# Sue1347/SMSUT-MedicalImgSegmentation

Measured on AMD Instinct MI355X. Metric: slices/sec uganConsisTrainer step @256x256, higher is better.
Workload: dtype f32

## Files before the change

include/smsut_hip.h:

```cpp
#ifndef SMSUT_HIP_H
#define SMSUT_HIP_H

#include <stdint.h>

#ifdef __cplusplus
extern "C" {
#endif

int smsut_conv2d_fwd_generic(const float* x, const float* w, const float* bias , float* y, int N, int H,
                             int W, int Cin, int Ho, int Wo, int Cout, int KH, int KW, int stride, int pad,
                             void* stream);
int smsut_conv2d_dgrad_generic(const float* gy, const float* w, float* gx, int N, int H, int W, int Cin, int Ho, int Wo,
                               int Cout, int KH, int KW, int stride, int pad, void* stream);
int64_t smsut_conv2d_wgrad_generic_ws(int N, int Ho, int Wo, int Cin, int Cout, int KH, int KW);
int smsut_conv2d_wgrad_generic(const float* x, const float* gy, float* gw, float* workspace, int N, int H, int W,
                               int Cin, int Ho, int Wo, int Cout, int KH, int KW, int stride, int pad, void* stream);

int smsut_conv2d_mfma_supported(int KS, int stride, int pad, int Kdim, int Ndim);
int smsut_conv2d_fwd_mfma(const float* x, const float* w, float* y, int N, int H, int W, int Kdim, int Ndim, int KS,
                          int transposed, void* stream);
int smsut_conv2d_mfma_tiles(int N, int H, int W, int Kdim, int Ndim, int KS, int f16);
int smsut_conv2d_mfma_persistent(int N, int H, int W, int Kdim, int Ndim, int KS, int f16);
int smsut_conv2d_dgrad_mfma_bwdstats(const float* gy, const float* w, float* gz, float* stats, const float* y1,
                                     const float* mean, const float* rstd, const float* gamma, const float* beta,
                                     float slope, int N, int H, int W, int Kdim, int Ndim, void* stream);
int smsut_conv2d_fwd_mfma_stats(const float* x, const float* w, float* y, float* stats, int N, int H, int W, int Kdim,
                                int Ndim, int KS, void* stream);
int smsut_conv2d_fwd_mfma_cfg(const float* x, const float* w, float* y, int N, int H, int W, int Kdim, int Ndim, int KS,
                              int transposed, int cfg, void* stream);
int64_t smsut_wino_image_floats(int Kdim, int Ndim);
int smsut_wino_prepare(const float* const* w, float* const* u, const int* Kdim, const int* Ndim, const int* transposed, int count,
                       void* stream);
int smsut_conv2d_fwd_mfma_pre(const float* x, const float* w, float* y, int N, int H, int W, int Kdim, int Ndim, int KS,
                              int transposed, const float* wu, void* stream);
int smsut_conv2d_fwd_mfma_stats_pre(const float* x, const float* w, float* y, float* stats, int N, int H, int W, int Kdim,
                                    int Ndim, int KS, const float* wu, void* stream);
int smsut_conv2d_dgrad_mfma_bwdstats_pre(const float* gy, const float* w, float* gz, float* stats, const float* y1,
                                         const float* mean, const float* rstd, const float* gamma, const float* beta,
                                         float slope, int N, int H, int W, int Kdim, int Ndim, const float* wu, void* stream);
int smsut_conv2d_fwd_mfma_stats_inaff_pre(const float* x, const float* w, float* y, float* stats, const float* mean,
                                          const float* rstd, const float* gamma, const float* beta, float slope, int N, int H,
                                          int W, int Kdim, int Ndim, const float* wu, void* stream);
int smsut_conv2d_fwd_mfma_stats_cat_pre(const float* xa, const float* xb, const float* w, float* y, float* stats, int N, int H,
                                        int W, int Kdim, int Ndim, const float* wu, void* stream);
int smsut_conv2d_fwd_mfma_split_pre(const float* x, const float* w, float* ya, float* yb, int split, int N, int H, int W,
                                    int Kdim, int Ndim, int transposed, const float* wu, void* stream);
int smsut_conv2d_fwd_mfma_stats_sc_pre(const float* x, const float* xb, const float* w, const float* wsc, float* y, float* ysc,
                                       float* stats, float* stats_sc, int N, int H, int W, int Kdim, int Ndim, const float* wu,
                                       void* stream);
int smsut_conv2d_wgrad_mfma_supported(int KS, int stride, int pad, int Cin, int Cout);
int64_t smsut_conv2d_wgrad_mfma_ws(int N, int H, int W, int Cin, int Cout, int KS);
int smsut_conv2d_wgrad_mfma(const float* x, const float* gy, float* gw, float* workspace, int N, int H, int W, int Cin,
                            int Cout, int KS, void* stream);

int smsut_conv1x1_supported(int Kdim, int Ndim);
int smsut_conv1x1_tiles(int N, int HW, int Ndim);
int smsut_conv1x1_fwd(const float* x, const float* w, float* y, float* stats , int N, int HW, int Kdim,
                      int Ndim, int transposed, void* stream);
int64_t smsut_conv1x1_wgrad_ws(int N, int HW, int Cin, int Cout);
int smsut_conv1x1_wgrad(const float* x, const float* gy, float* gw, float* workspace, int N, int HW, int Cin, int Cout,
                        void* stream);

int smsut_conv2d_fwd_mfma_stats_inaff(const float* x, const float* w, float* y, float* stats, const float* mean,
                                      const float* rstd, const float* gamma, const float* beta, float slope, int N, int H,
                                      int W, int Kdim, int Ndim, void* stream);
int smsut_conv2d_wgrad_mfma_inaff(const float* x, const float* gy, float* gw, float* workspace, const float* mean,
                                  const float* rstd, const float* gamma, const float* beta, float slope, int N, int H, int W,
                                  int Cin, int Cout, void* stream);
int smsut_conv2d_wgrad_mfma_slabs(const float* x, const float* gy, float* workspace, const float* mean, const float* rstd,
                                  const float* gamma, const float* beta, float slope, int N, int H, int W, int Cin, int Cout,
                                  void* stream);
int smsut_conv2d_mfma_form(int N, int H, int W, int Kdim, int Ndim, int sc_dgrad);

int smsut_conv2d_mfma_cat_supported(int N, int H, int W, int Kdim, int Ndim);
int smsut_conv2d_fwd_mfma_stats_cat(const float* xa, const float* xb, const float* w, float* y, float* stats, int N, int H,
                                    int W, int Kdim, int Ndim, void* stream);
int smsut_conv2d_fwd_sc_supported(int N, int H, int W, int Kdim, int Ndim, int cat);
int smsut_conv2d_fwd_mfma_stats_sc(const float* x, const float* xb , const float* w, const float* wsc, float* y,
                                   float* ysc, float* stats, float* stats_sc, int N, int H, int W, int Kdim, int Ndim,
                                   void* stream);
int smsut_conv2d_fwd_sc_f16_supported(int N, int H, int W, int Kdim, int Ndim, int cat);
int smsut_conv2d_fwd_mfma_stats_sc_f16(const float* x, const float* xb, const float* w, const float* wsc, float* y, float* ysc,
                                       float* stats, float* stats_sc, int N, int H, int W, int Kdim, int Ndim, void* stream);
int smsut_conv2d_dgrad_sc_supported(int N, int H, int W, int Cout, int Cin, int split);
int smsut_conv2d_dgrad_mfma_sc(const float* gy, const float* gs, const float* w, const float* wsc, float* gxa,
                               float* gxb , int split, int N, int H, int W, int Cout, int Cin, void* stream);
int smsut_conv2d_wgrad_sc_supported(int N, int H, int W, int Cin, int Cout);
int64_t smsut_conv2d_wgrad_sc_ws(int N, int H, int W, int Cin, int Cout);
int smsut_conv2d_wgrad_mfma_sc(const float* xa, const float* xb , int ca, const float* gy, const float* gs,
                               float* gw10, float* workspace, int N, int H, int W, int Cin, int Cout, void* stream);
int smsut_conv2d_wgrad_mfma_cat(const float* xa, const float* xb, int ca, const float* gy, float* gw, float* workspace,
                                int N, int H, int W, int Cin, int Cout, int KS, void* stream);
int smsut_conv2d_fwd_mfma_stats_sc_fin(const float* x, const float* xb , const float* w, const float* wsc, float* y,
                                       float* ysc, float* stats, float* stats_sc, int* tickets, float* mean, float* rstd,
                                       float* mean_sc, float* rstd_sc, float eps, int N, int H, int W, int Kdim, int Ndim,
                                       const float* wu , void* stream);
int smsut_conv2d_fwd_mfma_stats_inaff_fin(const float* x, const float* w, float* y, float* stats, const float* mean,
                                          const float* rstd, const float* gamma, const float* beta, float slope, int* tickets,
                                          float* mean_out, float* rstd_out, float eps, int N, int H, int W, int Kdim, int Ndim,
                                          const float* wu , void* stream);
int smsut_conv2d_dgrad_mfma_bwdstats_fin(const float* gy, const float* w, float* gz, float* stats, const float* y1,
                                         const float* mean, const float* rstd, const float* gamma, const float* beta, float slope,
                                         int* tickets, float* a_mean, float* b_mean, int N, int H, int W, int Kdim, int Ndim,
                                         const float* wu , void* stream);
int smsut_conv2d_wgrad_pair_supported(int NA, int NB, int H, int W, int Cin, int Cout, int cat, int aff, int sc);
int64_t smsut_conv2d_wgrad_pair_ws(int NA, int NB, int H, int W, int Cin, int Cout, int cat, int aff, int sc);
int smsut_conv2d_wgrad_pair(const float* xA, const float* x2A , const float* gyA, const float* gsA ,
                            const float* meanA , const float* rstdA , int NA, const float* xB,
                            const float* x2B , const float* gyB, const float* gsB ,
                            const float* meanB , const float* rstdB , int NB, int ca,
                            const float* gamma , const float* beta , float slope, float* gw, float* workspace,
                            int H, int W, int Cin, int Cout, void* stream);
int smsut_conv2d_wgrad_pair_slabs(const float* xA, const float* gyA, const float* meanA , const float* rstdA ,
                                  int NA, const float* xB, const float* gyB, const float* meanB ,
                                  const float* rstdB , int NB, const float* gamma , const float* beta ,
                                  float slope, float* workspace, int H, int W, int Cin, int Cout, void* stream);
int smsut_conv1x1_fwd_cat(const float* xa, const float* xb, int ca, const float* w, float* y, float* stats ,
                          int N, int HW, int Kdim, int Ndim, void* stream);
int smsut_conv1x1_wgrad_cat(const float* xa, const float* xb, int ca, const float* gy, float* gw, float* workspace, int N,
                            int HW, int Cin, int Cout, void* stream);

int smsut_conv2d_mfma_split_supported(int N, int H, int W, int Kdim, int Ndim, int split);
int smsut_conv2d_fwd_mfma_split(const float* x, const float* w, float* ya, float* yb, int split, int N, int H, int W,
                                int Kdim, int Ndim, int transposed, void* stream);
int smsut_conv1x1_fwd_split(const float* x, const float* w, float* ya, float* yb, int split, int N, int HW, int Kdim,
                            int Ndim, int transposed, void* stream);

int smsut_conv2d_f16_supported(int KS, int Kdim, int Ndim);
int smsut_conv2d_fwd_mfma_f16(const float* x, const float* w, float* y, const float* gsc , int N, int H, int W,
                              int Kdim, int Ndim, int KS, int transposed, void* stream);
int smsut_conv2d_fwd_mfma_stats_f16(const float* x, const float* w, float* y, float* stats, int N, int H, int W, int Kdim,
                                    int Ndim, int KS, void* stream);
int smsut_conv2d_fwd_mfma_stats_cat_f16(const float* xa, const float* xb, const float* w, float* y, float* stats, int N, int H,
                                        int W, int Kdim, int Ndim, void* stream);
int smsut_conv2d_fwd_mfma_split_f16(const float* x, const float* w, float* ya, float* yb, const float* gsc ,
                                    int split, int N, int H, int W, int Kdim, int Ndim, int transposed, void* stream);
int smsut_conv2d_f16_hs_supported(int N, int H, int W, int Kdim, int Ndim, int cat);
int smsut_conv2d_fwd_mfma_stats_f16_hs(const float* x, const float* xb , const float* w, void* y16, float* stats, int N,
                                       int H, int W, int Kdim, int Ndim, void* stream);
int smsut_conv2d_fwd_mfma_stats_f16_hsx(const void* x16, const float* w, void* y16, float* stats, int N, int H, int W, int Kdim,
                                        int Ndim, void* stream);
int smsut_conv2d_fwd_mfma_stats_inaff_f16_hsx(const void* y1_16, const float* w, void* y16, float* stats, const float* mean,
                                              const float* rstd, const float* gamma, const float* beta, float slope, int N, int H,
                                              int W, int Kdim, int Ndim, void* stream);
int smsut_conv2d_fwd_mfma_stats_sc_f16_hs(const float* x, const float* xb , const float* w, const float* wsc, void* y16,
                                          void* ysc16, float* stats, float* stats_sc, int N, int H, int W, int Kdim, int Ndim,
                                          void* stream);
int smsut_conv2d_dgrad_mfma_bwdstats_f16_hs(const float* gy, const float* w, float* gz, float* stats, const void* y1_16,
                                            const float* mean, const float* rstd, const float* gamma, const float* beta,
                                            const float* gsc , float slope, int N, int H, int W, int Kdim, int Ndim,
                                            void* stream);
int smsut_conv2d_dgrad_sc_f16_supported(int N, int H, int W, int Cout, int Cin, int split);
int smsut_conv2d_dgrad_mfma_sc_f16(const float* gy, const float* gs, const float* w, const float* wsc, float* gxa,
                                   float* gxb , const float* gsc, int split, int N, int H, int W, int Cout, int Cin,
                                   void* stream);
int smsut_conv2d_dgrad_mfma_bwdstats_f16(const float* gy, const float* w, float* gz, float* stats, const float* y1,
                                         const float* mean, const float* rstd, const float* gamma, const float* beta,
                                         const float* gsc , float slope, int N, int H, int W, int Kdim, int Ndim,
                                         void* stream);
int smsut_conv2d_wgrad_f16_supported(int N, int H, int W, int Cin, int Cout);
int64_t smsut_conv2d_wgrad_f16_ws(int N, int H, int W, int Cin, int Cout);
int smsut_conv2d_wgrad_f16(const float* x, const float* x2 , int ca, const float* gy, float* gw, float* workspace,
                           const float* gsc , int N, int H, int W, int Cin, int Cout, void* stream);
int smsut_conv2d_wgrad_f16_xh(const void* x16, const float* gy, float* gw, float* workspace, const float* gsc , int N,
                              int H, int W, int Cin, int Cout, void* stream);
int smsut_conv2d_wgrad_f16_xh_inaff(const void* y1_16, const float* gy, float* gw, float* workspace, const float* gsc ,
                                    const float* mean, const float* rstd, const float* gamma, const float* beta, float slope, int N,
                                    int H, int W, int Cin, int Cout, void* stream);
int smsut_conv2d_wgrad_sc_f16_supported(int N, int H, int W, int Cin, int Cout);
int64_t smsut_conv2d_wgrad_sc_f16_ws(int N, int H, int W, int Cin, int Cout);
int smsut_conv2d_wgrad_sc_f16(const float* x, const float* x2 , int ca, const float* gy, const float* gs, float* gw10,
                              float* workspace, const float* gsc, int N, int H, int W, int Cin, int Cout, void* stream);
int64_t smsut_absmax_scale_ws(int64_t n);
int smsut_absmax_scale(const float* x, int64_t n, float* out2, float* workspace, void* stream);
int smsut_absmax_scale2(const float* x, int64_t n, const float* x2, int64_t n2, float* out2, float* workspace, void* stream);
int smsut_absmax_finish(const float* amax, int n, float* out2, void* stream);

int smsut_conv2d_k4_supported(int Cin, int Cout);
int smsut_conv2d_k4_fwd(const float* x, const float* w, float* y, int N, int H, int W, int Cin, int Cout, int transposed,
                        void* stream);
int64_t smsut_conv2d_k4_wgrad_ws(int N, int H, int W, int Cin, int Cout);
int smsut_conv2d_k4_wgrad(const float* x, const float* gy, float* gw, float* workspace, int N, int H, int W, int Cin, int Cout,
                          void* stream);

int smsut_conv1x1_thin_supported(int Cin, int Cout);
int smsut_conv1x1_thin_dgrad(const float* gy, const float* w, float* gx, int N, int HW, int Cin, int Cout, void* stream);
int64_t smsut_conv1x1_thin_wgrad_ws(int Cin);
int smsut_conv1x1_thin_wgrad(const float* x, const float* gy, float* gw, float* workspace, int N, int HW, int Cin,
                             int Cout, void* stream);

int smsut_conv2d_small_supported(int KS, int Cin, int Cout);
int smsut_conv2d_small_fwd(const float* x, const float* w, const float* bias , float* y, int N, int H, int W,
                           int Cin, int Ho, int Wo, int Cout, int KS, int stride, int pad, void* stream);
int smsut_conv2d_small_dgrad(const float* gy, const float* w, float* gx, int N, int H, int W, int Cin, int Ho, int Wo,
                             int Cout, int KS, int stride, int pad, void* stream);
int smsut_conv2d_flat_wgrad_supported(int KS, int stride, int Cin, int Cout);
int64_t smsut_conv2d_flat_wgrad_ws(int N, int Ho, int Wo, int Cin, int Cout, int KS);
int smsut_conv2d_flat_wgrad(const float* x, const float* gy, float* gw, float* workspace, int N, int H, int W, int Cin,
                            int Ho, int Wo, int Cout, int KS, int stride, int pad, void* stream);

int smsut_convT2x2_mfma_supported(int Cin, int Cout);
int smsut_convT2x2_fwd_mfma(const float* x, const float* w, float* y, int N, int H, int W, int Cin, int Cout, void* stream);
int smsut_convT2x2_dgrad_mfma(const float* gy, const float* w, float* gx, int N, int H, int W, int Cin, int Cout,
                              void* stream);
int64_t smsut_convT2x2_wgrad_mfma_ws(int N, int H, int W, int Cin, int Cout);
int smsut_convT2x2_wgrad_mfma(const float* x, const float* gy, float* gw, float* workspace, int N, int H, int W, int Cin,
                              int Cout, void* stream);
int smsut_convT2x2_ps_supported(int Cin, int Cout);
int smsut_convT2x2_fwd_ps(const float* x, const float* w, float* y, int N, int H, int W, int Cin, int Cout, void* stream);
int64_t smsut_convT2x2_wgrad_ps_ws(int N, int H, int W, int Cin, int Cout);
int smsut_convT2x2_wgrad_ps(const float* x, const float* gy, float* gw, float* workspace, int N, int H, int W, int Cin,
                            int Cout, void* stream);

int64_t smsut_colsum_ws(int64_t rows, int C);
int smsut_colsum(const float* x, float* out, float* workspace, int64_t rows, int C, void* stream);

int smsut_in_chunks(int N, int HW, int C);
int smsut_in_slabs(int N, int HW, int C);
int smsut_instnorm_fwd(const float* x, const float* gamma, const float* beta, float* y, float* mean, float* rstd,
                       float* workspace, int N, int HW, int C, float eps, float slope, int has_act, void* stream);
int smsut_instnorm_fwd_partials(const float* x, const float* gamma, const float* beta, float* y, float* mean,
                                float* rstd, const float* partials, int chunks, int N, int HW, int C, float eps,
                                float slope, int has_act, void* stream);
int smsut_instnorm_fwd_partials_hs(const void* x16, const float* gamma, const float* beta, float* y, float* mean,
                                   float* rstd, const float* partials, int chunks, int N, int HW, int C, float eps,
                                   float slope, int has_act, void* stream);
int smsut_instnorm_fwd_partials_hs2(const void* x16, const float* gamma, const float* beta, void* y16, float* mean,
                                    float* rstd, const float* partials, int chunks, int N, int HW, int C, float eps,
                                    float slope, int has_act, void* stream);
int smsut_in_finalize_fwd(const float* partials, int chunks, float* mean, float* rstd, int N, int HW, int C, float eps,
                          void* stream);
int smsut_in_finalize_fwd2(const float* pa, int chunks_a, float* mean_a, float* rstd_a, const float* pb, int chunks_b, float* mean_b,
                           float* rstd_b, int N, int HW, int C, float eps, void* stream);
int smsut_in_finalize_bwd(const float* partials, int chunks, float* a_mean, float* b_mean, int N, int HW, int C, void* stream);
int smsut_in_apply_bwd(const float* gz, const float* x, const float* mean, const float* rstd, const float* gamma,
                       const float* a_mean, const float* b_mean, float* gx, float* ggamma ,
                       float* gbeta , int N, int HW, int C, void* stream);
int smsut_amax_blocks(int N, int HW, int C);
int smsut_in_apply_bwd_amax(const float* gz, const float* x, const float* mean, const float* rstd, const float* gamma,
                            const float* a_mean, const float* b_mean, float* gx, float* ggamma ,
                            float* gbeta , float* amax, int N, int HW, int C, void* stream);
int smsut_in_apply_bwd_hs(const float* gz, const void* x16, const float* mean, const float* rstd, const float* gamma,
                          const float* a_mean, const float* b_mean, float* gx, float* ggamma ,
                          float* gbeta , float* amax , int N, int HW, int C, void* stream);
int smsut_restail_fwd(const float* y2, const float* m2, const float* r2, const float* g2, const float* b2, const float* s,
                      const float* ms , const float* rs, const float* gs, const float* bs, float* out,
                      int N, int HW, int C, float slope, void* stream);
int smsut_restail_bwd(const float* gout, const float* out, const float* y2, const float* m2, const float* r2,
                      const float* g2, const float* b2 , const float* s, const float* ms ,
                      const float* rs, const float* gs_, const float* bs , float* gy2, float* gs, float* a_mean, float* b2_mean, float* bs_mean, float* gg2, float* gb2,
                      float* ggs , float* gbs , float* workspace, int N, int HW, int C,
                      float slope, void* stream);
int smsut_restail_bwd_fin(const float* gout, const float* out, const float* y2, const float* m2, const float* r2,
                      const float* g2, const float* b2 , const float* s, const float* ms ,
                      const float* rs, const float* gs_, const float* bs , float* gy2, float* gs, float* a_mean, float* b2_mean, float* bs_mean, float* gg2, float* gb2,
                      float* ggs , float* gbs , float* workspace, int* tickets, int N, int HW, int C,
                      float slope, void* stream);
int smsut_restail_fwd_hs(const void* y2_16, const float* m2, const float* r2, const float* g2, const float* b2, const void* s16,
                         const float* ms, const float* rs, const float* gs, const float* bs, float* out, int N, int HW, int C,
                         float slope, void* stream);
int smsut_restail_bwd_hs(const float* gout, const float* out, const void* y2_16, const float* m2, const float* r2,
                         const float* g2, const float* b2, const void* s16, const float* ms, const float* rs, const float* gs_,
                         const float* bs, float* gy2, float* gs, float* a_mean, float* b2_mean, float* bs_mean, float* gg2,
                         float* gb2, float* ggs, float* gbs, float* workspace, float* amax , int N, int HW, int C,
                         float slope, void* stream);
int smsut_restail_bwd_amax(const float* gout, const float* out, const float* y2, const float* m2, const float* r2,
                           const float* g2, const float* b2 , const float* s, const float* ms ,
                           const float* rs, const float* gs_, const float* bs , float* gy2, float* gs, float* a_mean, float* b2_mean, float* bs_mean, float* gg2, float* gb2,
                           float* ggs , float* gbs , float* workspace, float* amax, int N, int HW,
                           int C, float slope, void* stream);
int smsut_restail_fwd_pool(const void* y2, const float* m2, const float* r2, const float* g2, const float* b2, const void* s,
                           const float* ms, const float* rs, const float* gs, const float* bs, float* out, float* pooled,
                           void* idx , int N, int H, int W, int C, float slope, int hs, void* stream);
int smsut_restail_bwd_pool(const float* gout, const float* gp, const void* idx , const void* y2, const float* m2, const float* r2,
                           const float* g2, const float* b2, const void* s, const float* ms, const float* rs, const float* gs_,
                           const float* bs, float* gy2, float* gs, float* a_mean, float* b2_mean, float* bs_mean, float* gg2,
                           float* gb2, float* ggs, float* gbs, float* workspace, int* tickets , float* amax ,
                           int N, int H, int W, int C, float slope, int hs, void* stream);
int smsut_instnorm_bwd(const float* gy, const float* x, const float* beta , const float* mean,
                       const float* rstd, const float* gamma, float* gx, float* a_mean, float* b_mean,
                       float* ggamma , float* gbeta , float* workspace, int N, int HW, int C,
                       float slope, void* stream);
int smsut_instnorm_pool_fwd_partials(const float* x, const float* gamma, const float* beta, float* y, float* mean, float* rstd,
                                     const float* partials, int chunks, int N, int H, int W, int C, float eps, float slope,
                                     void* stream);
int smsut_instnorm_pool_bwd(const float* gyp, const float* x, const float* beta, const float* mean, const float* rstd,
                            const float* gamma, float* gx, float* a_mean, float* b_mean, float* ggamma ,
                            float* gbeta , float* workspace, int N, int H, int W, int C, float slope, void* stream);
int smsut_instnorm_bwd2(const float* v, const float* ug , const float* ub , const float* gy,
                        const float* x, const float* beta , const float* mean, const float* rstd,
                        const float* gamma, const float* a_mean, const float* b_mean, float* d_gy, float* d_x,
                        float* d_gamma, float* workspace, float* scratch , int N, int HW, int C, float slope,
                        void* stream);

int smsut_add_act(const float* a, const float* b , float* y, int64_t n, float slope, void* stream);
int smsut_act_bwd(const float* gy, const float* y, float* gx, int64_t n, float slope, void* stream);
int smsut_tanh_fwd(const float* x, float* y, int64_t n, void* stream);
int smsut_tanh_bwd(const float* gy, const float* y, float* gx, int64_t n, void* stream);
int smsut_bias_add(const float* x, const float* bias, float* y, int64_t rows, int C, void* stream);
int smsut_row_lerp(const float* a, const float* b, const float* alpha, float* out, int64_t rows, int64_t row_len,
                   void* stream);
int smsut_fill(float* out, float v, int64_t n, void* stream);
int smsut_scale(const float* x, const float* scale_dev , float mul, float* out, int64_t n, void* stream);
int smsut_sgd_momentum_multi(const void* ents, const int* blk_ent, const int* blk_chunk, int nblocks, float lr, float momentum, float wd,
                             void* stream);
int smsut_sgd_chunk(void);
int smsut_maxpool2_fwd(const float* x, float* y, int N, int H, int W, int C, void* stream);
int smsut_maxpool2_bwd(const float* gy, const float* x, float* gx, int N, int H, int W, int C, void* stream);
int smsut_maxpool2_bwd_add(const float* gy, const float* x, const float* add, float* gx, int N, int H, int W, int C,
                           void* stream);
int smsut_avgpool2_fwd(const float* x, float* y, int N, int H, int W, int C, void* stream);
int smsut_avgpool2_bwd(const float* gy, float* gx, int N, int H, int W, int C, void* stream);
int smsut_warp_joint(const float* img, const int64_t* msk, const float* aff, const float* ctrl, float* oimg,
                     int64_t* omsk, int N, int H, int W, int Ho, int Wo, int P, void* stream);
int smsut_elastic_deform(const float* img, const int64_t* msk, const float* coef, float* oimg, int64_t* omsk, int N, int H,
                         int W, int P, void* stream);
int smsut_photo_parts(int HW);
int smsut_photo_hist(const float* img, int* part, int N, int HW, void* stream);
int smsut_photo_apply(const float* img, const int* part , const float* params, const uint8_t* gtab ,
                      const float* out_tab, float* out, int N, int HW, void* stream);
int smsut_bilinear2_fwd(const float* x, float* y, int N, int H, int W, int C, void* stream);
int smsut_bilinear2_bwd(const float* gy, float* gx, int N, int H, int W, int C, void* stream);
int smsut_window_fwd(const float* src, float* dst, int N, int Hs, int Ws, int Hd, int Wd, int C, int oy, int ox, int mode,
                     void* stream);
int smsut_window_bwd(const float* gdst, float* gsrc, int N, int Hs, int Ws, int Hd, int Wd, int C, int oy, int ox, int mode,
                     void* stream);
int smsut_blurdown_fwd(const float* x, float* y, int N, int H, int W, int C, void* stream);
int smsut_blurdown_bwd(const float* gy, float* gx, int N, int H, int W, int C, void* stream);
int smsut_concat2(float* a, int Ca, float* b, int Cb, float* y, int64_t P, int dir, void* stream);
int smsut_copy_channels(const float* src, int Cs, int src_off, float* dst, int Cd, int dst_off, int Cc, int64_t P,
                        void* stream);
int smsut_modal_planes(const float* x, const float* m, float* out, int N, int64_t HW, int Cx, int M, void* stream);

int64_t smsut_dicece_ws(int N, int64_t HW, int C, int G);
int smsut_dicece_stats(const float* logits, const int64_t* labels, float* stats, float* ce_sum, float* workspace, int N,
                       int64_t HW, int C, int G, void* stream);
int smsut_dicece_final(const float* stats, const float* ce_sum, float* out , int G, int C, double npix_total,
                       float w_dc, float w_ce, void* stream);
int smsut_dicece_bwd(const float* logits, const int64_t* labels, const float* stats, const float* gout, float* glogits,
                     int N, int64_t HW, int C, int G, double npix_total, float w_dc, float w_ce, void* stream);
int64_t smsut_sum_ws(int64_t n, int rows);
int smsut_sum(const float* a, float* out, float* workspace, int64_t n, double scale, void* stream);
int smsut_l1_fwd(const float* a, const float* b, float* out, float* workspace, int64_t n, void* stream);
int smsut_l1_bwd(const float* a, const float* b, const float* gout, float* ga , float* gb ,
                 int64_t n, void* stream);
int smsut_softmax_mse_fwd(const float* a, const float* b, float* out, float* workspace, int64_t P, int C, void* stream);
int smsut_softmax_mse_bwd(const float* a, const float* b, const float* gout, float* ga, int64_t P, int C, void* stream);
int smsut_argmax_channels(const float* logits, int64_t* labels, int64_t P, int C, void* stream);
int smsut_gp_fwd(const float* dydx, float* out, float* norms, float* workspace, int rows, int64_t n, void* stream);
int smsut_gp_bwd(const float* dydx, const float* norms, const float* gout, float* g, int rows, int64_t n, void* stream);
int smsut_ce_rows_fwd(const float* z, const int64_t* tgt, float* out, int B, int C, void* stream);
int smsut_ce_rows_bwd(const float* z, const int64_t* tgt, const float* gout, float* gz, int B, int C, void* stream);
int smsut_gather_rows(const float* feat, const int64_t* ids, float* out, int B, int64_t HW, int C, int P, void* stream);
int smsut_scatter_rows(const float* gout, const int64_t* ids, float* gfeat, int B, int64_t HW, int C, int P,
                       void* stream);
int smsut_l2norm_fwd(const float* x, float* y, float* norms, int rows, int C, void* stream);
int smsut_l2norm_bwd(const float* gy, const float* x, const float* norms, float* gx, int rows, int C, void* stream);
int smsut_patchnce_fwd(const float* q, const float* k, float* loss, float* probs, int rows, int np, int dim, float T,
                       void* stream);
int smsut_patchnce_bwd(const float* gloss, const float* probs, const float* k, float* gq, int rows, int np, int dim,
                       float T, void* stream);

int64_t smsut_cora_ws(int N, int64_t HW, int L);
int smsut_cora_sup_stats(const float* logits, const int64_t* labels, const float* w_con, const float* w_rad, float* stats,
                         float* workspace, int N, int64_t HW, int L, void* stream);
int smsut_cora_sup_final(const float* stats, const float* w_con, const float* w_rad, float* out , int L, double npix_total,
                         float w_dc, float w_ce, void* stream);
int smsut_cora_sup_bwd(const float* logits, const int64_t* labels, const float* stats, const float* w_con, const float* w_rad,
                       const float* gout, float* glogits, int N, int64_t HW, int L, double npix_total, float w_dc, float w_ce,
                       void* stream);
int smsut_cora_semi_stats(const float* z, const float* e, const int64_t* q, const float* m, float* stats, float* workspace, int N,
                          int64_t HW, int L, void* stream);
int smsut_cora_semi_final(const float* stats, float* out , int N, int L, float cw, void* stream);
int smsut_cora_semi_bwd(const float* z, const float* e, const int64_t* q, const float* m, const float* stats, const float* gout ,
                        float* gz, int N, int64_t HW, int L, float cw, void* stream);
int smsut_cora_pseudo(const float* z, int64_t* q, float* m, int64_t P, int L, void* stream);
int smsut_ema_multi(const void* ents, const int* blk_ent, const int* blk_chunk, int nblocks, float alpha, float beta, void* stream);
int smsut_ema_chunk(void);

int64_t smsut_sdf_ws(int B, int C, int H, int W);
int smsut_edt_sq(const int64_t* labels, int* d2, float* workspace, int* status, int B, int C, int H, int W, void* stream);
int smsut_sdf_final(const int64_t* labels, const int* d2, const float* workspace, float* sdf, int B, int C, int H, int W, void* stream);
int64_t smsut_dtc_ws(int N, int64_t HW);
int smsut_dtc_loss_fwd(const float* t, const float* z, const float* sdf, float* out , float* workspace, int N, int B, int64_t HW,
                       int C, float k, void* stream);
int smsut_dtc_loss_bwd(const float* t, const float* z, const float* sdf, const float* gout , float* gt, float* gz, int N, int B,
                       int64_t HW, int C, float k, void* stream);

int64_t smsut_cc_ws(int D, int H, int W, int n_cls, int per_slice);
int smsut_cc_filter(const uint8_t* in, uint8_t* out, void* workspace, int D, int H, int W, int n_cls, int per_slice,
                    void* stream);
int64_t smsut_surface_ws(int D, int H, int W, int n_cls, int planar);
int smsut_surface_stats(const uint8_t* pred, const uint8_t* gt, double* out, void* workspace, int D, int H, int W, int n_cls,
                        int planar, void* stream);
int64_t smsut_surface_hd_ws(int D, int H, int W, int n_cls, int planar);
int smsut_surface_hd(const uint8_t* pred, const uint8_t* gt, double* out, void* workspace, int D, int H, int W, int n_cls,
                     int planar, double quantile, void* stream);
int64_t smsut_surface_sp_ws(int D, int H, int W, int n_cls, int planar);
int smsut_surface_stats_sp(const uint8_t* pred, const uint8_t* gt, double* out, void* workspace, int D, int H, int W, int n_cls,
                           int planar, double sz, double sy, double sx, void* stream);
int64_t smsut_surface_hd_sp_ws(int D, int H, int W, int n_cls, int planar);
int smsut_surface_hd_sp(const uint8_t* pred, const uint8_t* gt, double* out, void* workspace, int D, int H, int W, int n_cls,
                        int planar, double quantile, double sz, double sy, double sx, void* stream);
int smsut_eval_overlap(const float* logits, const int64_t* labels, const int* vol, int64_t* counts, uint8_t* pred , int N,
                       int64_t HW, int C, int K, int V, void* stream);
int64_t smsut_image_similarity_ws(int n, int h, int w);
int smsut_image_similarity(const float* a, const float* b, double* out, void* workspace, int n, int h, int w, double data_range,
                           void* stream);

int64_t smsut_bspline_ws(int d, int h, int w);
int smsut_bspline_coefficients(const float* vol, float* out, void* workspace, int d, int h, int w, void* stream);
int64_t smsut_resample_ws(int od, int oh, int ow);
int smsut_resample_volume(const float* coef, float* out, void* workspace, int sd, int sh, int sw, int od, int oh, int ow, int num_z,
                          int num_y, int num_x, int den_z, int den_y, int den_x, int start_z, int start_y, int start_x, int off_z,
                          int off_y, int off_x, void* stream);
int smsut_resample_labels(const uint8_t* lab, uint8_t* out, void* workspace, const uint8_t* lut , int sd, int sh, int sw,
                          int od, int oh, int ow, int num_z, int num_y, int num_x, int den_z, int den_y, int den_x, int start_z,
                          int start_y, int start_x, int off_z, int off_y, int off_x, void* stream);
int64_t smsut_order_statistics_ws(int64_t n, int nr);
int smsut_order_statistics(const float* v, float* out, void* workspace, int64_t n, int nr, int64_t r0, int64_t r1, int64_t r2,
                           int64_t r3, int64_t r4, int64_t r5, int64_t r6, int64_t r7, void* stream);
int smsut_window_u8(const float* v, const float* bounds, uint8_t* out, int64_t n, void* stream);

#define SMSUT_TTA_MAX_MEMBERS 16
#define SMSUT_TTA_MAX_CLASSES 32
#define SMSUT_TTA_MAX_SLICES 65535
#define SMSUT_TTA_MAX_DIM 16384
int smsut_tta_expand(const uint8_t* img, float* out, const int* transforms, int T, int N, int H, int W, void* stream);
int smsut_tta_merge(const float* const* members, const int* transforms, uint8_t* pred, float* conf ,
                    float* prob , int T, int N, int H, int W, int C, int K, void* stream);
int smsut_tta_uncertain(const float* const* members, const int* transforms, uint8_t* pred, float* conf ,
                        float* entropy , float* mutual , uint8_t* votes ,
                        int64_t* counts , int T, int N, int H, int W, int C, int K, void* stream);

#define SMSUT_CALIB_MAX_CLASSES 32
#define SMSUT_CALIB_MAX_BINS 64
#define SMSUT_CALIB_MAX_SLICES 65535
#define SMSUT_CALIB_MAX_DIM 16384
int64_t smsut_calibration_ws(int N, int H, int W, int C, int K, int B);
int smsut_calibration_stats(const float* logits, const int64_t* labels, double* out, void* workspace, int N, int H, int W, int C,
                            int K, int B, float beta, void* stream);

#ifdef __cplusplus
}
#endif
#endif
```

smsut-medicalimgsegmentation_amd/_hip.py:

```python
from __future__ import annotations

import ctypes
import os
from typing import Dict, Optional

import torch

_HERE = os.path.dirname(os.path.abspath(__file__))
LIB_PATH = os.path.join(_HERE, "lib", "libsmsut_hip.so")

SIGNATURES: Dict[str, str] = {
    "smsut_in_chunks": "iii",
    "smsut_in_slabs": "iii",
    "smsut_instnorm_fwd": "ppppppp iii ff i s",
    "smsut_instnorm_fwd_partials": "ppppppp iiii ff i s",
    "smsut_instnorm_fwd_partials_hs": "ppppppp iiii ff i s",
    "smsut_instnorm_fwd_partials_hs2": "ppppppp iiii ff i s",
    "smsut_in_finalize_fwd": "p i pp iii f s",
    "smsut_in_finalize_fwd2": "p i pp p i pp iii f s",
    "smsut_in_finalize_bwd": "p i pp iii s",
    "smsut_in_apply_bwd": "pppppppp pp iii s",
    "smsut_restail_fwd": "pppppppppp p iii f s",
    "smsut_restail_fwd_hs": "pppppppppp p iii f s",
    "smsut_restail_bwd_hs": "pppppppppppp pp ppp pppp pp iii f s",
    "smsut_in_apply_bwd_hs": "pppppppp pp p iii s",
    "smsut_restail_bwd": "pppppppppppp pp ppp pppp p iii f s",
    "smsut_restail_bwd_fin": "pppppppppppp pp ppp pppp pp iii f s",
    "smsut_restail_bwd_amax": "pppppppppppp pp ppp pppp pp iii f s",
    "smsut_in_apply_bwd_amax": "pppppppp pp p iii s",
    "smsut_absmax_scale_ws": "l",
    "smsut_absmax_scale": "p l pp s",
    "smsut_absmax_scale2": "p l p l pp s",
    "smsut_absmax_finish": "p i p s",
    "smsut_amax_blocks": "iii",
    "smsut_instnorm_bwd": "pppppp ppppp p iii f s",
    "smsut_restail_fwd_pool": "pppppppppp ppp iiii f i s",
    "smsut_restail_bwd_pool": "ppp pppppppppp pp ppp pppp p pp iiii f i s",
    "smsut_instnorm_pool_fwd_partials": "ppppppp iiiii ff s",
    "smsut_instnorm_pool_bwd": "pppppp ppppp p iiii f s",
    "smsut_instnorm_bwd2": "ppppppppppp ppp pp iii f s",
    "smsut_conv2d_fwd_generic": "pppp iiiiiiiiiii s",
    "smsut_conv2d_dgrad_generic": "ppp iiiiiiiiiii s",
    "smsut_conv2d_wgrad_generic_ws": "iiiiiii",
    "smsut_conv2d_wgrad_generic": "pppp iiiiiiiiiii s",
    "smsut_colsum_ws": "li",
    "smsut_colsum": "ppp li s",
    "smsut_conv2d_mfma_supported": "iiiii",
    "smsut_conv2d_fwd_mfma": "ppp iiiiii i s",
    "smsut_conv2d_fwd_mfma_pre": "ppp iiiiii i p s",
    "smsut_conv2d_mfma_tiles": "iiiiiii",
    "smsut_conv2d_mfma_persistent": "iiiiiii",
    "smsut_conv2d_dgrad_mfma_bwdstats": "ppppppppp f iiiii s",
    "smsut_conv2d_dgrad_mfma_bwdstats_pre": "ppppppppp f iiiii p s",
    "smsut_conv2d_fwd_mfma_stats": "pppp iiiiii s",
    "smsut_conv2d_fwd_mfma_stats_pre": "pppp iiiiii p s",
    "smsut_conv2d_fwd_mfma_cfg": "ppp iiiiii ii s",
    "smsut_convT2x2_mfma_supported": "ii",
    "smsut_convT2x2_fwd_mfma": "ppp iiiii s",
    "smsut_convT2x2_dgrad_mfma": "ppp iiiii s",
    "smsut_conv2d_fwd_mfma_stats_inaff": "pppp pppp f iiiii s",
    "smsut_conv2d_fwd_mfma_stats_inaff_pre": "pppp pppp f iiiii p s",
    "smsut_conv2d_mfma_form": "iiiiii",
    "smsut_conv2d_mfma_cat_supported": "iiiii",
    "smsut_conv2d_fwd_mfma_stats_cat": "ppppp iiiii s",
    "smsut_conv2d_fwd_mfma_stats_cat_pre": "ppppp iiiii p s",
    "smsut_conv2d_fwd_sc_supported": "iiiiii",
    "smsut_conv2d_fwd_mfma_stats_sc": "pppppppp iiiii s",
    "smsut_conv2d_fwd_mfma_stats_sc_f16": "pppppppp iiiii s",
    "smsut_conv2d_fwd_sc_f16_supported": "iiiiii",
    "smsut_conv2d_fwd_mfma_stats_sc_pre": "pppppppp iiiii p s",
    "smsut_conv2d_dgrad_sc_supported": "iiiiii",
    "smsut_conv2d_dgrad_mfma_sc": "pppppp iiiiii s",
    "smsut_conv2d_fwd_mfma_stats_sc_fin": "pppppppp ppppp f iiiii p s",
    "smsut_conv2d_fwd_mfma_stats_inaff_fin": "pppppppp f ppp f iiiii p s",
    "smsut_conv2d_dgrad_mfma_bwdstats_fin": "ppppppppp f ppp iiiii p s",
    "smsut_conv2d_k4_supported": "ii",
    "smsut_conv2d_k4_fwd": "ppp iiiii i s",
    "smsut_conv2d_f16_supported": "iii",
    "smsut_conv2d_fwd_mfma_f16": "pppp iiiiii i s",
    "smsut_conv2d_fwd_mfma_stats_f16": "pppp iiiiii s",
    "smsut_conv2d_fwd_mfma_stats_cat_f16": "ppppp iiiii s",
    "smsut_conv2d_fwd_mfma_split_f16": "ppppp iiiiiii s",
    "smsut_conv2d_dgrad_mfma_bwdstats_f16": "pppppppppp f iiiii s",
    "smsut_conv2d_dgrad_mfma_bwdstats_f16_hs": "pppppppppp f iiiii s",
    "smsut_conv2d_f16_hs_supported": "iiiiii",
    "smsut_conv2d_fwd_mfma_stats_f16_hs": "ppppp iiiii s",
    "smsut_conv2d_fwd_mfma_stats_f16_hsx": "pppp iiiii s",
    "smsut_conv2d_fwd_mfma_stats_inaff_f16_hsx": "pppp pppp f iiiii s",
    "smsut_conv2d_fwd_mfma_stats_sc_f16_hs": "pppppppp iiiii s",
    "smsut_conv2d_dgrad_sc_f16_supported": "iiiiii",
    "smsut_conv2d_dgrad_mfma_sc_f16": "ppppppp iiiiii s",
    "smsut_conv2d_mfma_split_supported": "iiiiii",
    "smsut_conv2d_fwd_mfma_split": "pppp iiiiiii s",
    "smsut_conv2d_fwd_mfma_split_pre": "pppp iiiiiii p s",
    "smsut_conv2d_wgrad_mfma_supported": "iiiii",
    "smsut_conv2d_wgrad_mfma_ws": "iiiiii",
    "smsut_conv2d_wgrad_mfma": "pppp iiiiii s",
    "smsut_convT2x2_wgrad_mfma_ws": "iiiii",
    "smsut_convT2x2_wgrad_mfma": "pppp iiiii s",
    "smsut_conv2d_wgrad_mfma_inaff": "pppp pppp f iiiii s",
    "smsut_conv2d_wgrad_mfma_slabs": "ppp pppp f iiiii s",
    "smsut_conv2d_wgrad_sc_supported": "iiiii",
    "smsut_conv2d_wgrad_sc_ws": "iiiii",
    "smsut_conv2d_wgrad_mfma_sc": "pp i pppp iiiii s",
    "smsut_conv2d_wgrad_mfma_cat": "pp i ppp iiiiii s",
    "smsut_conv2d_wgrad_pair_supported": "iiiiiiiii",
    "smsut_conv2d_wgrad_pair_ws": "iiiiiiiii",
    "smsut_conv2d_wgrad_pair": "pppppp i pppppp i i pp f pp iiii s",
    "smsut_conv2d_wgrad_pair_slabs": "pppp i pppp i pp f p iiii s",
    "smsut_conv2d_k4_wgrad_ws": "iiiii",
    "smsut_conv2d_k4_wgrad": "pppp iiiii s",
    "smsut_conv2d_wgrad_f16_xh": "ppppp iiiii s",
    "smsut_conv2d_wgrad_f16_xh_inaff": "ppppp pppp f iiiii s",
    "smsut_conv2d_wgrad_f16_supported": "iiiii",
    "smsut_conv2d_wgrad_f16_ws": "iiiii",
    "smsut_conv2d_wgrad_f16": "pp i pppp iiiii s",
    "smsut_conv2d_wgrad_sc_f16_supported": "iiiii",
    "smsut_conv2d_wgrad_sc_f16_ws": "iiiii",
    "smsut_conv2d_wgrad_sc_f16": "pp i ppppp iiiii s",
    "smsut_wino_image_floats": "ii",
    "smsut_wino_prepare": "ppppp i s",
    "smsut_convT2x2_ps_supported": "ii",
    "smsut_convT2x2_fwd_ps": "ppp iiiii s",
    "smsut_convT2x2_wgrad_ps_ws": "iiiii",
    "smsut_convT2x2_wgrad_ps": "pppp iiiii s",
    "smsut_conv1x1_supported": "ii",
    "smsut_conv1x1_tiles": "iii",
    "smsut_conv1x1_fwd": "pppp iiii i s",
    "smsut_conv1x1_wgrad_ws": "iiii",
    "smsut_conv1x1_wgrad": "pppp iiii s",
    "smsut_conv1x1_fwd_cat": "pp i ppp iiii s",
    "smsut_conv1x1_wgrad_cat": "pp i ppp iiii s",
    "smsut_conv1x1_fwd_split": "pppp iiiiii s",
    "smsut_conv1x1_thin_supported": "ii",
    "smsut_conv1x1_thin_dgrad": "ppp iiii s",
    "smsut_conv1x1_thin_wgrad_ws": "i",
    "smsut_conv1x1_thin_wgrad": "pppp iiii s",
    "smsut_conv2d_small_supported": "iii",
    "smsut_conv2d_small_fwd": "pppp iiiiiiiiii s",
    "smsut_conv2d_small_dgrad": "ppp iiiiiiiiii s",
    "smsut_conv2d_flat_wgrad_supported": "iiii",
    "smsut_conv2d_flat_wgrad_ws": "iiiiii",
    "smsut_conv2d_flat_wgrad": "pppp iiiiiiiiii s",
    "smsut_add_act": "ppp l f s",
    "smsut_act_bwd": "ppp l f s",
    "smsut_tanh_fwd": "pp l s",
    "smsut_tanh_bwd": "ppp l s",
    "smsut_bias_add": "ppp l i s",
    "smsut_row_lerp": "pppp ll s",
    "smsut_fill": "p f l s",
    "smsut_scale": "pp f p l s",
    "smsut_maxpool2_fwd": "pp iiii s",
    "smsut_maxpool2_bwd": "ppp iiii s",
    "smsut_maxpool2_bwd_add": "pppp iiii s",
    "smsut_avgpool2_fwd": "pp iiii s",
    "smsut_avgpool2_bwd": "pp iiii s",
    "smsut_bilinear2_fwd": "pp iiii s",
    "smsut_warp_joint": "pppppp iiiiii s",
    "smsut_elastic_deform": "ppppp iiii s",
    "smsut_bilinear2_bwd": "pp iiii s",
    "smsut_window_fwd": "pp iiiiiiiii s",
    "smsut_window_bwd": "pp iiiiiiiii s",
    "smsut_blurdown_fwd": "pp iiii s",
    "smsut_blurdown_bwd": "pp iiii s",
    "smsut_copy_channels": "p ii p ii i l s",
    "smsut_concat2": "p i p i p l i s",
    "smsut_modal_planes": "ppp i l ii s",
    "smsut_sgd_momentum_multi": "ppp i fff s",
    "smsut_sgd_chunk": "",
    "smsut_photo_parts": "i",
    "smsut_photo_hist": "pp ii s",
    "smsut_photo_apply": "pppppp ii s",
    "smsut_dicece_ws": "i l ii",
    "smsut_dicece_stats": "ppppp i l ii s",
    "smsut_dicece_final": "ppp ii d ff s",
    "smsut_dicece_bwd": "ppppp i l ii d ff s",
    "smsut_sum_ws": "l i",
    "smsut_sum": "ppp l d s",
    "smsut_l1_fwd": "pppp l s",
    "smsut_l1_bwd": "ppppp l s",
    "smsut_softmax_mse_fwd": "pppp l i s",
    "smsut_softmax_mse_bwd": "pppp l i s",
    "smsut_argmax_channels": "pp l i s",
    "smsut_gp_fwd": "pppp i l s",
    "smsut_gp_bwd": "pppp i l s",
    "smsut_ce_rows_fwd": "ppp ii s",
    "smsut_ce_rows_bwd": "pppp ii s",
    "smsut_gather_rows": "ppp i l ii s",
    "smsut_scatter_rows": "ppp i l ii s",
    "smsut_l2norm_fwd": "ppp ii s",
    "smsut_l2norm_bwd": "pppp ii s",
    "smsut_patchnce_fwd": "pppp iii f s",
    "smsut_patchnce_bwd": "pppp iii f s",
    "smsut_cora_ws": "i l i",
    "smsut_cora_sup_stats": "pppppp i l i s",
    "smsut_cora_sup_final": "pppp i d ff s",
    "smsut_cora_sup_bwd": "ppppppp i l i d ff s",
    "smsut_cora_semi_stats": "pppppp i l i s",
    "smsut_cora_semi_final": "pp ii f s",
    "smsut_cora_semi_bwd": "ppppppp i l i f s",
    "smsut_cora_pseudo": "ppp l i s",
    "smsut_ema_multi": "ppp i ff s",
    "smsut_ema_chunk": "",
    "smsut_sdf_ws": "iiii",
    "smsut_edt_sq": "pppp iiii s",
    "smsut_sdf_final": "pppp iiii s",
    "smsut_dtc_ws": "i l",
    "smsut_dtc_loss_fwd": "ppppp ii l i f s",
    "smsut_dtc_loss_bwd": "pppppp ii l i f s",
    "smsut_cc_ws": "iiiii",
    "smsut_cc_filter": "ppp iiiii s",
    "smsut_surface_ws": "iiiii",
    "smsut_surface_stats": "pppp iiiii s",
    "smsut_surface_hd_ws": "iiiii",
    "smsut_surface_hd": "pppp iiiii d s",
    "smsut_surface_sp_ws": "iiiii",
    "smsut_surface_stats_sp": "pppp iiiii ddd s",
    "smsut_surface_hd_sp_ws": "iiiii",
    "smsut_surface_hd_sp": "pppp iiiii d ddd s",
    "smsut_eval_overlap": "ppppp i l iii s",
    "smsut_image_similarity_ws": "iii",
    "smsut_image_similarity": "pppp iii d s",
    "smsut_bspline_ws": "iii",
    "smsut_bspline_coefficients": "ppp iii s",
    "smsut_resample_ws": "iii",
    "smsut_resample_volume": "ppp iii iii iii iii iii iii s",
    "smsut_resample_labels": "pppp iii iii iii iii iii iii s",
    "smsut_order_statistics_ws": "l i",
    "smsut_order_statistics": "ppp l i llllllll s",
    "smsut_window_u8": "ppp l s",
    "smsut_tta_expand": "ppp iiii s",
    "smsut_tta_merge": "ppppp iiiiii s",
    "smsut_tta_uncertain": "pppppppp iiiiii s",
    "smsut_calibration_ws": "iiiiii",
    "smsut_calibration_stats": "pppp iiiiii f s",
}
_RET_I64 = {"smsut_wino_image_floats", "smsut_conv2d_wgrad_pair_ws", "smsut_convT2x2_wgrad_ps_ws", "smsut_conv2d_wgrad_sc_ws", "smsut_conv2d_k4_wgrad_ws", "smsut_conv2d_wgrad_f16_ws", "smsut_conv2d_wgrad_sc_f16_ws", "smsut_absmax_scale_ws", "smsut_conv2d_wgrad_generic_ws", "smsut_colsum_ws", "smsut_dicece_ws", "smsut_sum_ws",
            "smsut_conv2d_wgrad_mfma_ws", "smsut_convT2x2_wgrad_mfma_ws", "smsut_conv2d_flat_wgrad_ws", "smsut_conv1x1_wgrad_ws",
            "smsut_conv1x1_thin_wgrad_ws", "smsut_cc_ws", "smsut_surface_ws", "smsut_surface_hd_ws", "smsut_surface_sp_ws", "smsut_surface_hd_sp_ws", "smsut_cora_ws",
            "smsut_sdf_ws", "smsut_dtc_ws", "smsut_image_similarity_ws",
            "smsut_bspline_ws", "smsut_resample_ws", "smsut_order_statistics_ws", "smsut_calibration_ws"}
_NO_STATUS = _RET_I64 | {"smsut_conv2d_k4_supported", "smsut_conv2d_f16_supported", "smsut_conv2d_wgrad_f16_supported", "smsut_in_chunks", "smsut_in_slabs", "smsut_amax_blocks", "smsut_conv2d_mfma_supported", "smsut_conv2d_wgrad_mfma_supported",
                         "smsut_convT2x2_mfma_supported", "smsut_conv2d_small_supported",
                         "smsut_conv2d_flat_wgrad_supported", "smsut_conv2d_mfma_tiles", "smsut_conv2d_mfma_persistent", "smsut_conv1x1_supported",
                         "smsut_conv1x1_tiles", "smsut_conv1x1_thin_supported", "smsut_conv2d_mfma_split_supported", "smsut_conv2d_mfma_cat_supported",
                         "smsut_conv2d_fwd_sc_supported", "smsut_conv2d_fwd_sc_f16_supported", "smsut_conv2d_dgrad_sc_supported",
                         "smsut_conv2d_dgrad_sc_f16_supported", "smsut_conv2d_wgrad_sc_f16_supported", "smsut_conv2d_f16_hs_supported",
                         "smsut_conv2d_wgrad_sc_supported", "smsut_convT2x2_ps_supported", "smsut_conv2d_wgrad_pair_supported",
                         "smsut_conv2d_wgrad_mfma_slabs", "smsut_conv2d_wgrad_pair_slabs", "smsut_conv2d_mfma_form", "smsut_sgd_chunk", "smsut_ema_chunk",
                         "smsut_photo_parts"}

_CT = {"p": ctypes.c_void_p, "i": ctypes.c_int, "l": ctypes.c_int64, "f": ctypes.c_float, "d": ctypes.c_double,
       "s": ctypes.c_void_p}

_lib: Optional[ctypes.CDLL] = None


class SmsutHipError(RuntimeError):
    pass


def load() -> ctypes.CDLL:
    global _lib
    if _lib is not None:
        return _lib
    if not os.path.exists(LIB_PATH):
        raise SmsutHipError(
            f"HIP extension not built: {LIB_PATH} is missing. Run `python -c 'import __graft_entry__ as g; g.build()'` "
            "(hipcc --offload-arch=gfx950). There is no CPU fallback for the product path.")
    lib = ctypes.CDLL(LIB_PATH)
    for name, sig in SIGNATURES.items():
        fn = getattr(lib, name)
        fn.argtypes = [_CT[c] for c in sig.replace(" ", "")]
        fn.restype = ctypes.c_int64 if name in _RET_I64 else ctypes.c_int
    _lib = lib
    return lib


def stream_ptr() -> int:
    if not torch.cuda.is_available():
        raise SmsutHipError("SMSUT HIP ops need an MI355X (no HIP device visible; there is no CPU fallback)")
    return torch.cuda.current_stream().cuda_stream


def ptr(t: Optional[torch.Tensor]):
    if t is None:
        return None
    if not t.is_cuda:
        raise SmsutHipError("SMSUT HIP ops need tensors on a HIP device (no CPU fallback in the product path)")
    return t.data_ptr()


def call(name: str, *args):
    lib = load()
    conv = [ptr(a) if isinstance(a, torch.Tensor) or a is None else a for a in args]
    rc = getattr(lib, name)(*conv)
    if name in _NO_STATUS:
        return rc
    if rc != 0:
        raise SmsutHipError(f"{name} failed with status {rc}" + (" (invalid argument)" if rc == -1 else " (hipError_t)"))
    return rc
```

smsut-medicalimgsegmentation_amd/csrc/conv_small.hip:

```cpp
#include "common.h"

namespace {

typedef float f32x4 __attribute__((ext_vector_type(4)));
constexpr int TPB = 256;
constexpr int MAXW = 2048;

struct SmallGeom { int N, H, W, Cin, Ho, Wo, Cout, KS, stride, pad; };

template <int CQ>
__global__ void __launch_bounds__(TPB)
small_fwd(const float* __restrict__ x, const float* __restrict__ w, const float* __restrict__ bias,
          float* __restrict__ y, SmallGeom g, int64_t npix) {
  __shared__ float4 ws[MAXW / 4];
  const int wq = g.KS * g.KS * g.Cin * CQ;
  for (int i = threadIdx.x; i < wq; i += TPB) ws[i] = ((const float4*)w)[i];
  __syncthreads();
  for (int64_t p = (int64_t)blockIdx.x * TPB + threadIdx.x; p < npix; p += (int64_t)gridDim.x * TPB) {
    const int wo = (int)(p % g.Wo);
    const int64_t q = p / g.Wo;
    const int ho = (int)(q % g.Ho);
    const int n = (int)(q / g.Ho);
    float4 acc[CQ];
#pragma unroll
    for (int c = 0; c < CQ; ++c) acc[c] = bias ? ((const float4*)bias)[c] : make_float4(0.f, 0.f, 0.f, 0.f);
    const float* xn = x + (size_t)n * g.H * g.W * g.Cin;
    for (int kh = 0; kh < g.KS; ++kh) {
      const int hi = ho * g.stride - g.pad + kh;
      if (hi < 0 || hi >= g.H) continue;
      for (int kw = 0; kw < g.KS; ++kw) {
        const int wi = wo * g.stride - g.pad + kw;
        if (wi < 0 || wi >= g.W) continue;
        const float* xp = xn + ((size_t)hi * g.W + wi) * g.Cin;
        const float4* wp = ws + (size_t)(kh * g.KS + kw) * g.Cin * CQ;
        for (int ci = 0; ci < g.Cin; ++ci) {
          const float v = xp[ci];
#pragma unroll
          for (int c = 0; c < CQ; ++c) {
            const float4 wv = wp[ci * CQ + c];
            acc[c].x = fmaf(v, wv.x, acc[c].x); acc[c].y = fmaf(v, wv.y, acc[c].y);
            acc[c].z = fmaf(v, wv.z, acc[c].z); acc[c].w = fmaf(v, wv.w, acc[c].w);
          }
        }
      }
    }
    float4* yp = (float4*)(y + (size_t)p * (4 * CQ));
#pragma unroll
    for (int c = 0; c < CQ; ++c) yp[c] = acc[c];
  }
}

template <int CQ, bool S1 = false>
__global__ void __launch_bounds__(TPB)
small_dgrad(const float* __restrict__ gy, const float* __restrict__ w, float* __restrict__ gx, SmallGeom g,
            int64_t npix) {
  __shared__ float4 ws[MAXW / 4];
  const int wq = g.KS * g.KS * g.Cin * CQ;
  for (int i = threadIdx.x; i < wq; i += TPB) ws[i] = ((const float4*)w)[i];
  __syncthreads();
  for (int64_t p = (int64_t)blockIdx.x * TPB + threadIdx.x; p < npix; p += (int64_t)gridDim.x * TPB) {
    const int wi = (int)(p % g.W);
    const int64_t q = p / g.W;
    const int hi = (int)(q % g.H);
    const int n = (int)(q / g.H);
    float acc[8];
#pragma unroll
    for (int c = 0; c < 8; ++c) acc[c] = 0.f;
    const float* gn = gy + (size_t)n * g.Ho * g.Wo * (4 * CQ);
    for (int kh = 0; kh < g.KS; ++kh) {
      const int hn = hi + g.pad - kh;
      if (hn < 0 || (!S1 && hn % g.stride)) continue;
      const int ho = S1 ? hn : hn / g.stride;
      if (ho >= g.Ho) continue;
      for (int kw = 0; kw < g.KS; ++kw) {
        const int wn = wi + g.pad - kw;
        if (wn < 0 || (!S1 && wn % g.stride)) continue;
        const int wo = S1 ? wn : wn / g.stride;
        if (wo >= g.Wo) continue;
        const float4* gp = (const float4*)(gn + ((size_t)ho * g.Wo + wo) * (4 * CQ));
        float4 gv[CQ];
#pragma unroll
        for (int c = 0; c < CQ; ++c) gv[c] = gp[c];
        const float4* wp = ws + (size_t)(kh * g.KS + kw) * g.Cin * CQ;
#pragma unroll
        for (int ci = 0; ci < 8; ++ci) {
          if (ci < g.Cin) {
#pragma unroll
            for (int c = 0; c < CQ; ++c) {
              const float4 wv = wp[ci * CQ + c];
              acc[ci] = fmaf(gv[c].x, wv.x, acc[ci]); acc[ci] = fmaf(gv[c].y, wv.y, acc[ci]);
              acc[ci] = fmaf(gv[c].z, wv.z, acc[ci]); acc[ci] = fmaf(gv[c].w, wv.w, acc[ci]);
            }
          }
        }
      }
    }
    float* op = gx + (size_t)p * g.Cin;
#pragma unroll
    for (int ci = 0; ci < 8; ++ci)
      if (ci < g.Cin) op[ci] = acc[ci];
  }
}

constexpr int FTH = 8, FTW = 16;
constexpr int MAXT = 4096;

template <int MT>
__global__ void __launch_bounds__(TPB)
flat_wgrad(const float* __restrict__ x, const float* __restrict__ gy, float* __restrict__ part, SmallGeom g,
           int tiles_x, int tiles_y, int tiles_per_split) {
  __shared__ float in_s[MAXT];
  __shared__ float gy_s[FTH * FTW * 16];
  __shared__ float red[MT * 64 * 4];
  const int tid = threadIdx.x, lane = tid & 63, wave = tid >> 6;
  const int lm = lane & 15, kq = lane >> 4;
  const int IH = (FTH - 1) * g.stride + g.KS, IW = (FTW - 1) * g.stride + g.KS;
  const int Mtot = g.KS * g.KS * g.Cin;
  int moff[MT];
#pragma unroll
  for (int i = 0; i < MT; ++i) {
    const int m = i * 16 + lm;
    const int tap = m / g.Cin, ci = m % g.Cin;
    moff[i] = m < Mtot ? ((tap / g.KS) * IW + (tap % g.KS)) * g.Cin + ci : -1;
  }
  f32x4 acc[MT];
#pragma unroll
  for (int i = 0; i < MT; ++i) acc[i] = (f32x4){0.f, 0.f, 0.f, 0.f};

  const int tiles_img = tiles_x * tiles_y;
  const int total = g.N * tiles_img;
  const int t0 = blockIdx.x * tiles_per_split;
  const int t1 = min(t0 + tiles_per_split, total);
  for (int t = t0; t < t1; ++t) {
    const int n = t / tiles_img, rem = t % tiles_img;
    const int oy0 = (rem / tiles_x) * FTH, ox0 = (rem % tiles_x) * FTW;
    const int iy0 = oy0 * g.stride - g.pad, ix0 = ox0 * g.stride - g.pad;
    const float* xn = x + (size_t)n * g.H * g.W * g.Cin;
    const float* gn = gy + (size_t)n * g.Ho * g.Wo * g.Cout;
    __syncthreads();
    for (int u = tid; u < IH * IW * g.Cin; u += TPB) {
      const int ci = u % g.Cin, pix = u / g.Cin;
      const int iy = iy0 + pix / IW, ix = ix0 + pix % IW;
      in_s[u] = (iy >= 0 && iy < g.H && ix >= 0 && ix < g.W) ? xn[((size_t)iy * g.W + ix) * g.Cin + ci] : 0.f;
    }
    for (int u = tid; u < FTH * FTW * 16; u += TPB) {
      const int c = u & 15, pix = u >> 4;
      const int oy = oy0 + pix / FTW, ox = ox0 + pix % FTW;
      gy_s[u] = (c < g.Cout && oy < g.Ho && ox < g.Wo) ? gn[((size_t)oy * g.Wo + ox) * g.Cout + c] : 0.f;
    }
    __syncthreads();
#pragma unroll
    for (int rr = 0; rr < FTH / 4; ++rr) {
      const int r = wave * (FTH / 4) + rr;
#pragma unroll
      for (int ks = 0; ks < FTW / 4; ++ks) {
        const int px = ks * 4 + kq;
        const float b = gy_s[(r * FTW + px) * 16 + lm];
        const int base = (r * g.stride * IW + px * g.stride) * g.Cin;
#pragma unroll
        for (int i = 0; i < MT; ++i) {
          const float a = moff[i] >= 0 ? in_s[base + moff[i]] : 0.f;
          acc[i] = __builtin_amdgcn_mfma_f32_16x16x4f32(a, b, acc[i], 0, 0, 0);
        }
      }
    }
  }
  for (int src = 1; src < 4; ++src) {
    __syncthreads();
    if (wave == src) {
#pragma unroll
      for (int i = 0; i < MT; ++i) *(f32x4*)(red + ((size_t)i * 64 + lane) * 4) = acc[i];
    }
    __syncthreads();
    if (wave == 0) {
#pragma unroll
      for (int i = 0; i < MT; ++i) acc[i] += *(const f32x4*)(red + ((size_t)i * 64 + lane) * 4);
    }
  }
  if (wave == 0) {
    float* out = part + (size_t)blockIdx.x * Mtot * g.Cout;
#pragma unroll
    for (int i = 0; i < MT; ++i)
#pragma unroll
      for (int r = 0; r < 4; ++r) {
        const int m = i * 16 + 4 * kq + r;
        if (m < Mtot && lm < g.Cout) out[(size_t)m * g.Cout + lm] = acc[i][r];
      }
  }
}

constexpr int FS_COLS = 4;
__global__ void __launch_bounds__(TPB)
flat_sum(const float* __restrict__ part, float* __restrict__ out, int wsize, int splits) {
  constexpr int LANES = TPB / FS_COLS;
  __shared__ double sm[TPB];
  const int col = threadIdx.x % FS_COLS, sl = threadIdx.x / FS_COLS;
  const int e = blockIdx.x * FS_COLS + col;
  double s0 = 0.0, s1 = 0.0, s2 = 0.0, s3 = 0.0;
  if (e < wsize) {
    int c = sl;
    for (; c + 3 * LANES < splits; c += 4 * LANES) {
      s0 += (double)part[(size_t)c * wsize + e];
      s1 += (double)part[(size_t)(c + LANES) * wsize + e];
      s2 += (double)part[(size_t)(c + 2 * LANES) * wsize + e];
      s3 += (double)part[(size_t)(c + 3 * LANES) * wsize + e];
    }
    for (; c < splits; c += LANES) s0 += (double)part[(size_t)c * wsize + e];
  }
  sm[threadIdx.x] = (s0 + s1) + (s2 + s3);
  __syncthreads();
  if (sl == 0 && e < wsize) {
    double t = 0.0;
    for (int l = 0; l < LANES; ++l) t += sm[l * FS_COLS + col];
    out[e] = (float)t;
  }
}

constexpr int STY = 16, STX = 64, SKS = 5, SPD = 2, SCO = 8;
constexpr int SIH = STY + SKS - 1, SIW = STX + SKS - 1;

template <int CIN>
__device__ __forceinline__ void stem_stage(const float* __restrict__ x, float* __restrict__ in_s, int n, int y0, int x0,
                                           int H, int W) {
  for (int u = threadIdx.x; u < SIH * SIW * CIN; u += TPB) {
    const int ci = u % CIN, pix = u / CIN;
    const int iy = pix / SIW, ix = pix % SIW;
    const int gy_ = y0 + iy - SPD, gx_ = x0 + ix - SPD;
    float v = 0.f;
    if (gy_ >= 0 && gy_ < H && gx_ >= 0 && gx_ < W) v = x[(((size_t)n * H + gy_) * W + gx_) * CIN + ci];
    in_s[(ci * SIH + iy) * SIW + ix] = v;
  }
}

template <int CIN>
__global__ void __launch_bounds__(TPB)
stem_fwd(const float* __restrict__ x, const float* __restrict__ w, const float* __restrict__ bias, float* __restrict__ y,
         int N, int H, int W) {
  __shared__ __attribute__((aligned(16))) float in_s[CIN * SIH * SIW];
  __shared__ __attribute__((aligned(16))) float w_s[SKS * SKS * CIN * SCO];
  const int tiles_x = W / STX, tiles_y = H / STY;
  const int t = blockIdx.x;
  const int n = t / (tiles_x * tiles_y), rem = t % (tiles_x * tiles_y);
  const int y0 = (rem / tiles_x) * STY, x0 = (rem % tiles_x) * STX;
  for (int u = threadIdx.x; u < SKS * SKS * CIN * SCO; u += TPB) w_s[u] = w[u];
  stem_stage<CIN>(x, in_s, n, y0, x0, H, W);
  __syncthreads();
  const int row = threadIdx.x >> 4, cg = threadIdx.x & 15;
  float acc[4][SCO];
#pragma unroll
  for (int p = 0; p < 4; ++p)
#pragma unroll
    for (int c = 0; c < SCO; ++c) acc[p][c] = bias ? bias[c] : 0.f;
#pragma unroll
  for (int kh = 0; kh < SKS; ++kh)
#pragma unroll
    for (int ci = 0; ci < CIN; ++ci) {
      float v[8];
      const float* ip = in_s + (ci * SIH + row + kh) * SIW + 4 * cg;
      *(float4*)v = *(const float4*)ip; *(float4*)(v + 4) = *(const float4*)(ip + 4);
#pragma unroll
      for (int kw = 0; kw < SKS; ++kw) {
        float wv[SCO];
        const float* wp = w_s + ((kh * SKS + kw) * CIN + ci) * SCO;
        *(float4*)wv = *(const float4*)wp; *(float4*)(wv + 4) = *(const float4*)(wp + 4);
#pragma unroll
        for (int p = 0; p < 4; ++p)
#pragma unroll
          for (int c = 0; c < SCO; ++c) acc[p][c] = fmaf(v[p + kw], wv[c], acc[p][c]);
      }
    }
  float* yp = y + (((size_t)n * H + y0 + row) * W + x0 + 4 * cg) * SCO;
#pragma unroll
  for (int p = 0; p < 4; ++p) {
    *(float4*)(yp + p * SCO) = *(float4*)acc[p];
    *(float4*)(yp + p * SCO + 4) = *(float4*)(acc[p] + 4);
  }
}

__global__ void __launch_bounds__(TPB)
stem_dgrad1(const float* __restrict__ gy, const float* __restrict__ w, float* __restrict__ gx, int N, int H, int W) {
  __shared__ __attribute__((aligned(16))) float g_s[SCO * SIH * SIW];
  __shared__ __attribute__((aligned(16))) float w_s[SKS * SKS * SCO];
  const int tiles_x = W / STX, tiles_y = H / STY;
  const int t = blockIdx.x;
  const int n = t / (tiles_x * tiles_y), rem = t % (tiles_x * tiles_y);
  const int y0 = (rem / tiles_x) * STY, x0 = (rem % tiles_x) * STX;
  for (int u = threadIdx.x; u < SKS * SKS * SCO; u += TPB) w_s[u] = w[u];
  for (int u = threadIdx.x; u < SIH * SIW * 2; u += TPB) {
    const int h = u & 1, pix = u >> 1;
    const int iy = pix / SIW, ix = pix % SIW;
    const int gy_ = y0 + iy - SPD, gx_ = x0 + ix - SPD;
    float4 v = make_float4(0.f, 0.f, 0.f, 0.f);
    if (gy_ >= 0 && gy_ < H && gx_ >= 0 && gx_ < W) v = *(const float4*)(gy + (((size_t)n * H + gy_) * W + gx_) * SCO + 4 * h);
    float* d = g_s + ((4 * h) * SIH + iy) * SIW + ix;
    d[0] = v.x; d[SIH * SIW] = v.y; d[2 * SIH * SIW] = v.z; d[3 * SIH * SIW] = v.w;
  }
  __syncthreads();
  const int row = threadIdx.x >> 4, cg = threadIdx.x & 15;
  float acc[4] = {0.f, 0.f, 0.f, 0.f};
#pragma unroll
  for (int jh = 0; jh < SKS; ++jh)
#pragma unroll
    for (int co = 0; co < SCO; ++co) {
      float v[8];
      const float* ip = g_s + (co * SIH + row + jh) * SIW + 4 * cg;
      *(float4*)v = *(const float4*)ip; *(float4*)(v + 4) = *(const float4*)(ip + 4);
#pragma unroll
      for (int jw = 0; jw < SKS; ++jw) {
        const float wv = w_s[((SKS - 1 - jh) * SKS + (SKS - 1 - jw)) * SCO + co];
#pragma unroll
        for (int p = 0; p < 4; ++p) acc[p] = fmaf(v[p + jw], wv, acc[p]);
      }
    }
  *(float4*)(gx + ((size_t)n * H + y0 + row) * W + x0 + 4 * cg) = *(float4*)acc;
}

constexpr int SGQ = 36;
template <int CIN>
__global__ void __launch_bounds__(TPB)
stem_wgrad(const float* __restrict__ x, const float* __restrict__ gy, float* __restrict__ part, int N, int H, int W,
           int tiles_per_wg) {
  extern __shared__ __attribute__((aligned(16))) float smem[];
  float* in_s = smem;
  float* gy_s = smem + CIN * SIH * SIW;
  constexpr int NACC = SKS * SCO;
  constexpr int TPP = (CIN == 1) ? 32 : 8;
  const int tiles_x = W / STX, tiles_y = H / STY, total = N * tiles_x * tiles_y;
  const int q = threadIdx.x / TPP, sub = threadIdx.x % TPP;
  const bool live = q < SKS * CIN;
  const int kh = q / CIN, k2 = q % CIN;
  float acc[NACC];
#pragma unroll
  for (int i = 0; i < NACC; ++i) acc[i] = 0.f;
  const int t0 = blockIdx.x * tiles_per_wg, t1 = min(t0 + tiles_per_wg, total);
  for (int t = t0; t < t1; ++t) {
    const int n = t / (tiles_x * tiles_y), rem = t % (tiles_x * tiles_y);
    const int y0 = (rem / tiles_x) * STY, x0 = (rem % tiles_x) * STX;
    __syncthreads();
    stem_stage<CIN>(x, in_s, n, y0, x0, H, W);
    for (int u = threadIdx.x; u < STY * (STX / 4) * 8; u += TPB) {
      const int half = u & 1, px = (u >> 1) & 3, quad = u >> 3;
      const int row = quad >> 4, cgq = quad & 15;
      *(float4*)(gy_s + quad * SGQ + px * SCO + 4 * half) =
          *(const float4*)(gy + (((size_t)n * H + y0 + row) * W + x0 + 4 * cgq + px) * SCO + 4 * half);
    }
    __syncthreads();
    if (live) {
      for (int k = 0; k < 256 / TPP; ++k) {
        const int quad = sub + TPP * k;
        const int row = quad >> 4, cgq = quad & 15;
        float g[4][SCO];
#pragma unroll
        for (int p = 0; p < 4; ++p) {
          *(float4*)g[p] = *(const float4*)(gy_s + quad * SGQ + p * SCO);
          *(float4*)(g[p] + 4) = *(const float4*)(gy_s + quad * SGQ + p * SCO + 4);
        }
        {
          float v[8];
          const float* ip = in_s + (k2 * SIH + row + kh) * SIW + 4 * cgq;
          *(float4*)v = *(const float4*)ip; *(float4*)(v + 4) = *(const float4*)(ip + 4);
#pragma unroll
          for (int kw = 0; kw < SKS; ++kw)
#pragma unroll
            for (int c = 0; c < SCO; ++c)
              acc[kw * SCO + c] += v[kw] * g[0][c] + v[kw + 1] * g[1][c] + v[kw + 2] * g[2][c] + v[kw + 3] * g[3][c];
        }
      }
    }
  }
#pragma unroll
  for (int i = 0; i < NACC; ++i) {
    float a = acc[i];
    a += __shfl_xor(a, 1, 64); a += __shfl_xor(a, 2, 64); a += __shfl_xor(a, 4, 64);
    if constexpr (TPP == 32) { a += __shfl_xor(a, 8, 64); a += __shfl_xor(a, 16, 64); }
    acc[i] = a;
  }
  if (live && sub == 0) {
    float* out = part + (size_t)blockIdx.x * SKS * SKS * CIN * SCO;
#pragma unroll
    for (int kw = 0; kw < SKS; ++kw)
#pragma unroll
      for (int c = 0; c < SCO; ++c) out[((kh * SKS + kw) * CIN + k2) * SCO + c] = acc[kw * SCO + c];
  }
}

inline bool stem_shape(const SmallGeom& g) {
  return g.KS == SKS && g.stride == 1 && g.pad == SPD && g.Cout == SCO && (g.Cin == 1 || g.Cin == 5) && g.H % STY == 0 &&
         g.W % STX == 0 && g.Ho == g.H && g.Wo == g.W;
}
inline int stem_wgrad_wgs(const SmallGeom& g, int max_slabs) {
  const int total = g.N * (g.H / STY) * (g.W / STX);
  int wgs = total < 512 ? total : 512;
  if (wgs > max_slabs) wgs = max_slabs;
  return wgs < 1 ? 1 : wgs;
}

inline bool geom_ok(const SmallGeom& g) {
  return g.N > 0 && g.H > 0 && g.W > 0 && g.Cin > 0 && g.Cout > 0 && g.KS > 0 && g.stride > 0 && g.pad >= 0 &&
         g.Ho == (g.H + 2 * g.pad - g.KS) / g.stride + 1 && g.Wo == (g.W + 2 * g.pad - g.KS) / g.stride + 1 && g.Ho > 0 &&
         g.Wo > 0;
}

struct FlatPlan { int tiles_x, tiles_y, splits, tiles_per_split; };
inline FlatPlan flat_plan(const SmallGeom& g) {
  FlatPlan p;
  p.tiles_x = (g.Wo + FTW - 1) / FTW;
  p.tiles_y = (g.Ho + FTH - 1) / FTH;
  const int total = g.N * p.tiles_x * p.tiles_y;
  int want = total < 2048 ? total : 2048;
  p.tiles_per_split = (total + want - 1) / want;
  p.splits = (total + p.tiles_per_split - 1) / p.tiles_per_split;
  return p;
}

}

extern "C" {

int smsut_conv2d_small_supported(int KS, int Cin, int Cout) {
  return KS >= 1 && Cin >= 1 && Cin <= 8 && Cout >= 4 && Cout <= 16 && (Cout % 4) == 0 && KS * KS * Cin * Cout <= MAXW;
}

int smsut_conv2d_small_fwd(const float* x, const float* w, const float* bias, float* y, int N, int H, int W, int Cin,
                           int Ho, int Wo, int Cout, int KS, int stride, int pad, void* stream) {
  SmallGeom g{N, H, W, Cin, Ho, Wo, Cout, KS, stride, pad};
  SMSUT_REQUIRE(x && w && y && geom_ok(g) && smsut_conv2d_small_supported(KS, Cin, Cout));
  const int64_t npix = (int64_t)N * Ho * Wo;
  const int grid = ew_grid(npix) * 2;
  hipStream_t st = (hipStream_t)stream;
  if (stem_shape(g)) {
    const int tiles = N * (H / STY) * (W / STX);
    if (Cin == 1) stem_fwd<1><<<tiles, TPB, 0, st>>>(x, w, bias, y, N, H, W);
    else stem_fwd<5><<<tiles, TPB, 0, st>>>(x, w, bias, y, N, H, W);
    SMSUT_LAUNCH_CHECK();
    return SMSUT_OK;
  }
  switch (Cout / 4) {
    case 1: small_fwd<1><<<grid, TPB, 0, st>>>(x, w, bias, y, g, npix); break;
    case 2: small_fwd<2><<<grid, TPB, 0, st>>>(x, w, bias, y, g, npix); break;
    case 3: small_fwd<3><<<grid, TPB, 0, st>>>(x, w, bias, y, g, npix); break;
    default: small_fwd<4><<<grid, TPB, 0, st>>>(x, w, bias, y, g, npix); break;
  }
  SMSUT_LAUNCH_CHECK();
  return SMSUT_OK;
}

int smsut_conv2d_small_dgrad(const float* gy, const float* w, float* gx, int N, int H, int W, int Cin, int Ho, int Wo,
                             int Cout, int KS, int stride, int pad, void* stream) {
  SmallGeom g{N, H, W, Cin, Ho, Wo, Cout, KS, stride, pad};
  SMSUT_REQUIRE(gy && w && gx && geom_ok(g) && smsut_conv2d_small_supported(KS, Cin, Cout));
  const int64_t npix = (int64_t)N * H * W;
  const int grid = ew_grid(npix) * 2;
  hipStream_t st = (hipStream_t)stream;
  if (stem_shape(g) && Cin == 1) {
    stem_dgrad1<<<N * (H / STY) * (W / STX), TPB, 0, st>>>(gy, w, gx, N, H, W);
    SMSUT_LAUNCH_CHECK();
    return SMSUT_OK;
  }
#define SMALL_DG(Q) do { if (stride == 1) small_dgrad<Q, true><<<grid, TPB, 0, st>>>(gy, w, gx, g, npix);  \
                         else small_dgrad<Q, false><<<grid, TPB, 0, st>>>(gy, w, gx, g, npix); } while (0)
  switch (Cout / 4) {
    case 1: SMALL_DG(1); break;
    case 2: SMALL_DG(2); break;
    case 3: SMALL_DG(3); break;
    default: SMALL_DG(4); break;
  }
#undef SMALL_DG
  SMSUT_LAUNCH_CHECK();
  return SMSUT_OK;
}

int smsut_conv2d_flat_wgrad_supported(int KS, int stride, int Cin, int Cout) {
  const int IH = (FTH - 1) * stride + KS, IW = (FTW - 1) * stride + KS;
  return KS >= 1 && stride >= 1 && Cin >= 1 && Cout >= 1 && Cout <= 16 && KS * KS * Cin <= 128 && IH * IW * Cin <= MAXT;
}

int64_t smsut_conv2d_flat_wgrad_ws(int N, int Ho, int Wo, int Cin, int Cout, int KS) {
  SmallGeom g{N, 0, 0, Cin, Ho, Wo, Cout, KS, 1, 0};
  return (int64_t)flat_plan(g).splits * KS * KS * Cin * Cout;
}

int smsut_conv2d_flat_wgrad(const float* x, const float* gy, float* gw, float* workspace, int N, int H, int W, int Cin,
                            int Ho, int Wo, int Cout, int KS, int stride, int pad, void* stream) {
  SmallGeom g{N, H, W, Cin, Ho, Wo, Cout, KS, stride, pad};
  SMSUT_REQUIRE(x && gy && gw && workspace && geom_ok(g) && smsut_conv2d_flat_wgrad_supported(KS, stride, Cin, Cout));
  const FlatPlan p = flat_plan(g);
  hipStream_t st = (hipStream_t)stream;
  if (stem_shape(g)) {
    const int wgs = stem_wgrad_wgs(g, p.splits);
    const int total = N * (H / STY) * (W / STX);
    const int tpw = (total + wgs - 1) / wgs;
    const int nwg = (total + tpw - 1) / tpw;
    const int wsz = KS * KS * Cin * Cout;
    if (Cin == 1) {
      constexpr size_t sh = (size_t)(1 * SIH * SIW + STY * (STX / 4) * SGQ) * sizeof(float);
      stem_wgrad<1><<<nwg, TPB, sh, st>>>(x, gy, workspace, N, H, W, tpw);
    } else {
      constexpr size_t sh = (size_t)(5 * SIH * SIW + STY * (STX / 4) * SGQ) * sizeof(float);
      static bool attr = false;
      if (!attr) { (void)hipFuncSetAttribute((const void*)stem_wgrad<5>, hipFuncAttributeMaxDynamicSharedMemorySize, (int)sh); attr = true; }
      stem_wgrad<5><<<nwg, TPB, sh, st>>>(x, gy, workspace, N, H, W, tpw);
    }
    flat_sum<<<(wsz + FS_COLS - 1) / FS_COLS, TPB, 0, st>>>(workspace, gw, wsz, nwg);
    SMSUT_LAUNCH_CHECK();
    return SMSUT_OK;
  }
  const int mt = (KS * KS * Cin + 15) / 16;
  if (mt <= 1) flat_wgrad<1><<<p.splits, TPB, 0, st>>>(x, gy, workspace, g, p.tiles_x, p.tiles_y, p.tiles_per_split);
  else if (mt <= 2) flat_wgrad<2><<<p.splits, TPB, 0, st>>>(x, gy, workspace, g, p.tiles_x, p.tiles_y, p.tiles_per_split);
  else if (mt <= 4) flat_wgrad<4><<<p.splits, TPB, 0, st>>>(x, gy, workspace, g, p.tiles_x, p.tiles_y, p.tiles_per_split);
  else flat_wgrad<8><<<p.splits, TPB, 0, st>>>(x, gy, workspace, g, p.tiles_x, p.tiles_y, p.tiles_per_split);
  const int wsize = KS * KS * Cin * Cout;
  flat_sum<<<(wsize + FS_COLS - 1) / FS_COLS, TPB, 0, st>>>(workspace, gw, wsize, p.splits);
  SMSUT_LAUNCH_CHECK();
  return SMSUT_OK;
}

}
```

smsut-medicalimgsegmentation_amd/network/ugan.py:

```python
import numpy as np
import torch
import torch.nn as nn

from .. import config as cfg
from .. import ops
from . import networks
from .blocks import (Act, BasicBlock, BottleBlock, Conv2d, MaxPool2x2, UpSampleAndConcat, encoder_level, get_act, get_norm,
                     init_conv_kaiming)


class _Pre(nn.Sequential):

    def forward(self, x):
        return self[1](self[0](x, stats=True), slope=self[2].slope)


class Encoder(nn.Module):
    def __init__(self, in_ch, base_width=32, norm_type="batch", act_type="relu"):
        super().__init__()
        w = base_width
        self.pre = _Pre(Conv2d(in_ch, w // 2, 5, stride=1, padding=2, bias=False), get_norm(w // 2, norm_type),
                        get_act(act_type))
        chans = [w // 2, w, 2 * w, 4 * w, 8 * w]
        for i in range(1, 5):
            setattr(self, f"enc{i}", BasicBlock(chans[i - 1], chans[i], norm_type, act_type))
            setattr(self, f"pool{i}", MaxPool2x2())

    def forward(self, x):
        skips = []
        x = self.pre(x)
        for i in range(1, 5):
            x, skip = encoder_level(getattr(self, f"enc{i}"), getattr(self, f"pool{i}"), x)
            skips.append(skip)
        skips.reverse()
        return x, skips


class Decoder(nn.Module):
    def __init__(self, out_ch, base_width=32, norm_type="batch", act_type="relu", tranposed=True, use_tanh=False):
        super().__init__()
        w = base_width
        for lvl, m in zip((4, 3, 2, 1), (8, 4, 2, 1)):
            setattr(self, f"up{lvl}", UpSampleAndConcat(2 * m * w, m * w, transposed=tranposed))
            setattr(self, f"dec{lvl}", BasicBlock(2 * m * w, m * w, norm_type, act_type))
        self.fc = Conv2d(w, out_ch, 1, bias=True)
        self.tanh = _Tanh() if use_tanh else None

    def forward(self, e5, x_ens):
        h = e5
        for i, lvl in enumerate((4, 3, 2, 1)):
            h = getattr(self, f"dec{lvl}")(getattr(self, f"up{lvl}")(h, x_ens[i]))
        out = self.fc(h)
        return self.tanh(out) if self.tanh is not None else out


class _Tanh(nn.Module):
    def forward(self, x):
        return ops.tanh(x)


class _UGANBase(nn.Module):
    def _build(self, in_ch, out_ch, n_modal, base_width, with_nce):
        self.n_modal = n_modal
        self.tsl_encoder = Encoder(in_ch + n_modal, base_width, norm_type="instance", act_type="lrelu")
        self.seg_encoder = Encoder(in_ch, base_width, norm_type="instance", act_type="lrelu")
        self.enc5 = BasicBlock(8 * base_width, 16 * base_width, norm="instance", act="lrelu")
        if with_nce:
            self.netF = define_F(in_ch)
            if not self.netF.mlp_init:
                self.netF.create_mlp(cfg.nce_layers)
        self.tsl_decoder = Decoder(1, base_width, norm_type="instance", act_type="lrelu", tranposed=False,
                                   use_tanh=True)
        self.seg_decoder = Decoder(out_ch, base_width, norm_type="instance", act_type="lrelu", tranposed=True,
                                   use_tanh=False)
        init_conv_kaiming(self, "leaky_relu")

    def _tsl_branch(self, x, m):
        if m is None:
            m = torch.zeros(x.size(0), self.n_modal, device=x.device)
        tsl_in = ops.modal_planes(x, m.to(x.device))
        t_bot, t_sk = self.tsl_encoder(tsl_in)
        t_e5 = self.enc5(t_bot)
        return self.tsl_decoder(t_e5, t_sk), t_e5

    def _seg_branch(self, x):
        s_bot, s_sk = self.seg_encoder(x)
        return self.seg_decoder(self.enc5(s_bot), s_sk)

    def _trunk(self, x, m):
        tsl, t_e5 = self._tsl_branch(x, m)
        return self._seg_branch(x), tsl, t_e5


class UGAN(_UGANBase):
    def __init__(self, in_ch, out_ch, n_modal, base_width=32):
        super().__init__()
        self._build(in_ch, out_ch, n_modal, base_width, with_nce=False)

    def forward(self, x, m=None):
        seg, tsl, _ = self._trunk(x, m)
        return seg, tsl


class UGANnce(_UGANBase):
    def __init__(self, in_ch, out_ch, n_modal, base_width=32, val_phase=False):
        super().__init__()
        self.val_phase = val_phase
        self._build(in_ch, out_ch, n_modal, base_width, with_nce=True)

    def forward(self, x, m=None, sample_ids=None, val_phase=False, branch=None):
        if branch == "seg":
            return self._seg_branch(x)
        if branch == "tsl":
            tsl, t_e5 = self._tsl_branch(x, m)
            if sample_ids is None:
                return tsl, None, None, t_e5
            feat_pool, _ = self.netF([t_e5], patch_ids=sample_ids)
            return tsl, feat_pool, sample_ids, t_e5
        seg, tsl, t_e5 = self._trunk(x, m)
        if val_phase:
            return seg, tsl
        feats = [t_e5]
        if sample_ids is None:
            feat_pool, sample_ids = self.netF(feats)
        else:
            feat_pool, _ = self.netF(feats, patch_ids=sample_ids)
        return seg, tsl, feat_pool, sample_ids


class Discriminator(nn.Module):
    def __init__(self, input_size, n_modal, base_width=32, max_width=512):
        super().__init__()
        layers = [Conv2d(1, base_width, 4, stride=2, padding=1, bias=True), Act(0.01)]
        repeat_num = int(np.log2(input_size)) - 2
        in_w = base_width
        out_w = base_width
        for _ in range(1, repeat_num):
            out_w = min(in_w * 2, max_width)
            layers.append(BottleBlock(in_w, out_w, norm_type="instance", act_type="lrelu", stride=2))
            in_w = out_w
        blocks_ = [m for m in layers if isinstance(m, BottleBlock)]
        for a, b in zip(blocks_[:-1], blocks_[1:]):
            a.feeds_stride2 = b.stride == 2
        self.main = nn.Sequential(*layers)
        k = int(input_size / np.power(2, repeat_num))
        self.conv_src = Conv2d(out_w, 1, 3, stride=1, padding=1, bias=False)
        self.conv_cls = Conv2d(out_w, n_modal, k, bias=False)
        init_conv_kaiming(self, "leaky_relu")

    def forward(self, x):
        h = self.main(x)
        out_src = self.conv_src(h)
        out_cls = self.conv_cls(h)
        return out_src, out_cls.reshape(out_cls.size(0), out_cls.size(1))


def define_F(input_nc, netF="mlp_sample", norm="batch", use_dropout=False, init_type="normal", init_gain=0.02,
             no_antialias=False, gpu_ids=None, netF_nc=256):
    net = PatchSampleF(use_mlp=True, init_type=init_type, init_gain=init_gain, gpu_ids=gpu_ids or [], nc=netF_nc)
    return init_net(net, init_type, init_gain, gpu_ids or [])


def init_net(net, init_type="normal", init_gain=0.02, gpu_ids=(), debug=False, initialize_weights=True):
    return networks.init_net(net, init_type, init_gain, gpu_ids, debug, initialize_weights)


class PatchSampleF(nn.Module):
    def __init__(self, use_mlp=False, init_type="normal", init_gain=0.02, nc=256, gpu_ids=()):
        super().__init__()
        self.l2norm = networks.Normalize(2)
        self.use_mlp = use_mlp
        self.nc = nc
        self.mlp_init = False
        self.init_type, self.init_gain, self.gpu_ids = init_type, init_gain, list(gpu_ids)

    def create_mlp(self, nce_layers, input_nc=256):
        for mlp_id, _ in enumerate(nce_layers):
            mlp = nn.Sequential(networks.Linear(input_nc, self.nc), networks.ReLU(), networks.Linear(self.nc, self.nc))
            setattr(self, "mlp_%d" % mlp_id, mlp)
        init_net(self, self.init_type, self.init_gain, self.gpu_ids)
        self.mlp_init = True

    def forward(self, feats, num_patches=64, patch_ids=None):
        return_ids, return_feats = [], []
        if self.use_mlp and not self.mlp_init:
            self.create_mlp(cfg.nce_layers)
        for feat_id, feat in enumerate(feats):
            hw = feat.shape[2] * feat.shape[3]
            if num_patches <= 0:
                raise NotImplementedError("num_patches=0 (dense) is not used by any trainer")
            if patch_ids is not None:
                patch_id = patch_ids[feat_id]
            else:
                patch_id = torch.randperm(hw, device=feat.device)[: int(min(num_patches, hw))]
            x_sample = ops.gather_patches(feat, patch_id.to(feat.device))
            if self.use_mlp:
                x_sample = getattr(self, "mlp_%d" % feat_id)(x_sample)
            return_ids.append(patch_id)
            return_feats.append(self.l2norm(x_sample))
        return return_feats, return_ids
```

smsut-medicalimgsegmentation_amd/ops.py:

```python
from __future__ import annotations

import contextlib
import math
import os as _os
from typing import NamedTuple, Optional

import torch
from torch.autograd import Function
from torch.autograd.function import once_differentiable

from . import _hip as H

IN_EPS = 1e-5

_INPUT_GRADS_ONLY = False


@contextlib.contextmanager
def input_grads_only():
    global _INPUT_GRADS_ONLY
    prev, _INPUT_GRADS_ONLY = _INPUT_GRADS_ONLY, True
    try:
        yield
    finally:
# ... 1300 lines not shown


class TanhFn(Function):
    @staticmethod
    def forward(ctx, x):
        x = nhwc(x)
        y = new_act(*x.shape, x)
        H.call("smsut_tanh_fwd", x, y, x.numel(), _s())
        ctx.save_for_backward(y)
        return y

    @staticmethod
    @once_differentiable
    def backward(ctx, gy):
        (y,) = ctx.saved_tensors
        gy = nhwc(gy)
        gx = new_act(*y.shape, y)
        H.call("smsut_tanh_bwd", gy, y, gx, y.numel(), _s())
        return gx


def tanh(x):
    return TanhFn.apply(x)


class MaxPool2Fn(Function):

    @staticmethod
    def forward(ctx, x):
        x = nhwc(x)
        n, c, h, w = x.shape
        y = new_act(n, c, h // 2, w // 2, x)
        H.call("smsut_maxpool2_fwd", x, y, n, h, w, c, _s())
        ctx.save_for_backward(x)
        return y

    @staticmethod
    @once_differentiable
    def backward(ctx, gy):
        (x,) = ctx.saved_tensors
        gy = nhwc(gy)
        n, c, h, w = x.shape
        gx = new_act(n, c, h, w, x)
        H.call("smsut_maxpool2_bwd", gy, x, gx, n, h, w, c, _s())
        return gx


class MaxPool2SkipFn(Function):

    @staticmethod
    def forward(ctx, x):
        x = nhwc(x)
        n, c, h, w = x.shape
        y = new_act(n, c, h // 2, w // 2, x)
        H.call("smsut_maxpool2_fwd", x, y, n, h, w, c, _s())
        ctx.save_for_backward(x)
        return y, x.view_as(x)

    @staticmethod
    @once_differentiable
    def backward(ctx, gy, gskip):
        (x,) = ctx.saved_tensors
        n, c, h, w = x.shape
        if gy is None:
            return gskip
        gy = nhwc(gy)
        gx = new_act(n, c, h, w, x)
        if gskip is None:
            H.call("smsut_maxpool2_bwd", gy, x, gx, n, h, w, c, _s())
        else:
            H.call("smsut_maxpool2_bwd_add", gy, x, nhwc(gskip), gx, n, h, w, c, _s())
        return gx


def max_pool2_skip(x):
    if x.is_cuda and x.requires_grad and torch.is_grad_enabled():
        return MaxPool2SkipFn.apply(x)
    return max_pool2(x), x


class AvgPool2Fn(Function):

    @staticmethod
    def forward(ctx, x):
        x = nhwc(x)
        n, c, h, w = x.shape
        y = new_act(n, c, h // 2, w // 2, x)
        H.call("smsut_avgpool2_fwd", x, y, n, h, w, c, _s())
        return y

    @staticmethod
    def backward(ctx, gy):
        return AvgPool2BwdFn.apply(gy)


class AvgPool2BwdFn(Function):
    @staticmethod
    def forward(ctx, gy):
        gy = nhwc(gy)
        n, c, ho, wo = gy.shape
        gx = new_act(n, c, 2 * ho, 2 * wo, gy)
        H.call("smsut_avgpool2_bwd", gy, gx, n, 2 * ho, 2 * wo, c, _s())
        return gx

    @staticmethod
    def backward(ctx, gg):
        return AvgPool2Fn.apply(gg)


class Bilinear2Fn(Function):

    @staticmethod
    def forward(ctx, x):
        x = nhwc(x)
        n, c, h, w = x.shape
        y = new_act(n, c, 2 * h, 2 * w, x)
        H.call("smsut_bilinear2_fwd", x, y, n, h, w, c, _s())
        return y

    @staticmethod
    @once_differentiable
    def backward(ctx, gy):
        gy = nhwc(gy)
        n, c, ho, wo = gy.shape
        gx = new_act(n, c, ho // 2, wo // 2, gy)
        H.call("smsut_bilinear2_bwd", gy, gx, n, ho // 2, wo // 2, c, _s())
        return gx


def max_pool2(x):
    return MaxPool2Fn.apply(x)


def avg_pool2(x):
    return AvgPool2Fn.apply(cl(x))


def bilinear_up2(x):
    return Bilinear2Fn.apply(x)


class WindowFn(Function):
    MODES = {"zero": 0, "reflect": 1, "refl": 1, "replicate": 2, "repl": 2}

    @staticmethod
    def forward(ctx, x, top, bottom, left, right, mode):
        x = nhwc(x)
        n, c, h, w = x.shape
        hd, wd = h + top + bottom, w + left + right
        y = new_act(n, c, hd, wd, x)
        H.call("smsut_window_fwd", x, y, n, h, w, hd, wd, c, top, left, mode, _s())
        ctx.geom = (h, w, hd, wd, top, left, mode)
        return y

    @staticmethod
    @once_differentiable
    def backward(ctx, gy):
        gy = nhwc(gy)
        h, w, hd, wd, top, left, mode = ctx.geom
        n, c = gy.shape[0], gy.shape[1]
        gx = new_act(n, c, h, w, gy)
        H.call("smsut_window_bwd", gy, gx, n, h, w, hd, wd, c, top, left, mode, _s())
        return gx, None, None, None, None, None


def pad2d(x, pads, mode="zero"):
    left, right, top, bottom = pads
    return WindowFn.apply(cl(x), top, bottom, left, right, WindowFn.MODES[mode])


class BlurDownFn(Function):

    @staticmethod
    def forward(ctx, x):
        x = nhwc(x)
        n, c, h, w = x.shape
        y = new_act(n, c, (h - 1) // 2 + 1, (w - 1) // 2 + 1, x)
        H.call("smsut_blurdown_fwd", x, y, n, h, w, c, _s())
        ctx.shape = (n, c, h, w)
        return y

    @staticmethod
    @once_differentiable
    def backward(ctx, gy):
        gy = nhwc(gy)
        n, c, h, w = ctx.shape
        gx = new_act(n, c, h, w, gy)
        H.call("smsut_blurdown_bwd", gy, gx, n, h, w, c, _s())
        return gx


def blur_down2(x):
    return BlurDownFn.apply(cl(x))


class ConcatFn(Function):

    @staticmethod
    def forward(ctx, a, b):
        a, b = nhwc(a), nhwc(b)
        n, ca, h, w = a.shape
        cb = b.shape[1]
        assert b.shape[0] == n and b.shape[2:] == a.shape[2:]
        y = new_act(n, ca + cb, h, w, a)
        p = n * h * w
        if ca % 4 == 0 and cb % 4 == 0:
            H.call("smsut_concat2", a, ca, b, cb, y, p, 0, _s())
        else:
            H.call("smsut_copy_channels", a, ca, 0, y, ca + cb, 0, ca, p, _s())
            H.call("smsut_copy_channels", b, cb, 0, y, ca + cb, ca, cb, p, _s())
        ctx.split = (ca, cb)
        return y

    @staticmethod
    @once_differentiable
    def backward(ctx, gy):
        gy = nhwc(gy)
        ca, cb = ctx.split
        n, _, h, w = gy.shape
        p = n * h * w
        ga = new_act(n, ca, h, w, gy) if ctx.needs_input_grad[0] else None
        gb = new_act(n, cb, h, w, gy) if ctx.needs_input_grad[1] else None
        if ca % 4 == 0 and cb % 4 == 0 and (ga is not None or gb is not None):
            H.call("smsut_concat2", ga, ca, gb, cb, gy, p, 1, _s())
        else:
            if ga is not None:
                H.call("smsut_copy_channels", gy, ca + cb, 0, ga, ca, 0, ca, p, _s())
            if gb is not None:
                H.call("smsut_copy_channels", gy, ca + cb, ca, gb, cb, 0, cb, p, _s())
        return ga, gb


def concat_channels(a, b):
    y = ConcatFn.apply(a, b)
    if SPLIT_DGRAD and torch.is_grad_enabled() and (a.requires_grad or b.requires_grad) and a.shape[1] % 16 == 0:
        y._smsut_cat_parts = (a, b)
    return y


class RowSegmentsFn(Function):

    @staticmethod
    def forward(ctx, y, *bounds):
        y = nhwc(y)
        ctx.shape, ctx.bounds = tuple(y.shape), tuple(int(b) for b in bounds)
        ctx.set_materialize_grads(False)
        return tuple(y[ctx.bounds[2 * i]:ctx.bounds[2 * i + 1]] for i in range(len(bounds) // 2))

    @staticmethod
    @once_differentiable
    def backward(ctx, *gs):
        n, c, h, w = ctx.shape
        ref = next(g for g in gs if g is not None)
        out = new_act(n, c, h, w, ref)
        pos = 0
        segs = sorted((ctx.bounds[2 * i], ctx.bounds[2 * i + 1], gs[i]) for i in range(len(gs)))
        for a, b, g in segs:
            if a > pos:
                out[pos:a].zero_()
            if g is None:
                out[a:b].zero_()
            else:
                out[a:b].copy_(g)
            pos = b
        if pos < n:
            out[pos:].zero_()
        return (out,) + (None,) * len(ctx.bounds)


def row_segments(y, *bounds):
    return RowSegmentsFn.apply(y, *bounds)


class ModalPlanesFn(Function):

    @staticmethod
    def forward(ctx, x, m):
        x = nhwc(x)
        n, cx, h, w = x.shape
        m = m.to(torch.float32).contiguous()
        nm = m.shape[1]
        y = new_act(n, cx + nm, h, w, x)
        H.call("smsut_modal_planes", x, m, y, n, h * w, cx, nm, _s())
        ctx.dims = (cx, nm)
        return y

    @staticmethod
    @once_differentiable
    def backward(ctx, gy):
        gy = nhwc(gy)
        cx, nm = ctx.dims
        n, _, h, w = gy.shape
        gx = None
        if ctx.needs_input_grad[0]:
            gx = new_act(n, cx, h, w, gy)
            H.call("smsut_copy_channels", gy, cx + nm, 0, gx, cx, 0, cx, n * h * w, _s())
        return gx, None


def modal_planes(x, m):
    return ModalPlanesFn.apply(x, m)


def dice_ce_stats(logits, labels, batch_dice):
    logits = nhwc(logits.detach())
    n, c, h, w = logits.shape
    labels = labels.contiguous()
    if labels.dtype != torch.int64:
        raise TypeError("labels must be int64")
    g = 1 if batch_dice else n
    stats = torch.empty(g, c, 3, dtype=torch.float32, device=logits.device)
    ce_sum = torch.empty(1, dtype=torch.float32, device=logits.device)
    H.call("smsut_dicece_stats", logits, labels, stats, ce_sum, _ws(H.call("smsut_dicece_ws", n, h * w, c, g), logits),
           n, h * w, c, g, _s())
    return stats, ce_sum


class DiceCEFromStatsFn(Function):

    @staticmethod
    def forward(ctx, logits, labels, stats, ce_sum, w_ce, w_dc, world):
        logits = nhwc(logits)
        n, c, h, w = logits.shape
        g = stats.shape[0]
        npix = float(n * h * w) * world
        out = torch.empty(3, dtype=torch.float32, device=logits.device)
        H.call("smsut_dicece_final", stats, ce_sum, out, g, c, npix, float(w_dc), float(w_ce), _s())
        ctx.save_for_backward(logits, labels.contiguous(), stats)
        ctx.cfg = (g, npix, float(w_dc), float(w_ce), int(world))
        return out[0]

    @staticmethod
    @once_differentiable
    def backward(ctx, gout):
        logits, labels, stats = ctx.saved_tensors
        g, npix, w_dc, w_ce, world = ctx.cfg
        n, c, h, w = logits.shape
        gl = new_act(n, c, h, w, logits)
        gout = gout.contiguous()
        if world > 1:
            gout = gout * float(world)
        H.call("smsut_dicece_bwd", logits, labels, stats, gout, gl, n, h * w, c, g, npix, w_dc, w_ce, _s())
        return gl, None, None, None, None, None, None


def dice_ce_from_stats(logits, labels, stats, ce_sum, weight_ce, weight_dc, world=1):
    return DiceCEFromStatsFn.apply(logits, labels, stats, ce_sum, weight_ce, weight_dc, world)


def all_reduce_dice_stats(pairs, group):
    import torch.distributed as dist
    from . import graphs
    graphs.assert_no_capture("all_reduce_dice_stats (Dice-statistics all-reduce)")
    ts = [t for pair in pairs for t in pair]
    adjacent = all(t.is_contiguous() for t in ts) and all(
        a.untyped_storage().data_ptr() == b.untyped_storage().data_ptr() and a.storage_offset() + a.numel() == b.storage_offset()
        for a, b in zip(ts, ts[1:]))
    if adjacent:
        span = ts[0].as_strided((sum(t.numel() for t in ts),), (1,), ts[0].storage_offset())
        dist.all_reduce(span, group=group)
        return
    flat = torch.cat([t.reshape(-1) for t in ts])
    dist.all_reduce(flat, group=group)
    off = 0
    for t in ts:
        n = t.numel()
        t.copy_(flat[off:off + n].view_as(t))
        off += n


class DiceCEFn:

    @staticmethod
    def apply(logits, labels, w_ce, w_dc, batch_dice, group):
        stats, ce_sum = dice_ce_stats(logits, labels, batch_dice)
        world = 1
        if group is not None and batch_dice:
            import torch.distributed as dist
            world = dist.get_world_size(group)
            if world > 1:
                all_reduce_dice_stats([(stats, ce_sum)], group)
        return DiceCEFromStatsFn.apply(logits, labels, stats, ce_sum, w_ce, w_dc, world)


def dice_ce(logits, labels, weight_ce=1.0, weight_dc=1.0, batch_dice=False, group=None):
    return DiceCEFn.apply(logits, labels, weight_ce, weight_dc, batch_dice, group)


class ScaledSumFn(Function):

    @staticmethod
    def forward(ctx, x, scale):
        x = x.contiguous() if x.dim() != 4 else nhwc(x)
        out = torch.empty(1, dtype=torch.float32, device=x.device)
        n = x.numel()
        H.call("smsut_sum", x, out, _ws(H.call("smsut_sum_ws", n, 1), x), n, float(scale), _s())
        ctx.meta = (x.shape, x.stride(), float(scale))
        return out[0]

    @staticmethod
    @once_differentiable
    def backward(ctx, gout):
        shape, stride, scale = ctx.meta
        gx = torch.empty_strided(shape, stride, dtype=torch.float32, device=gout.device)
        H.call("smsut_fill", gx, 1.0, gx.numel(), _s())
        out = torch.empty_strided(shape, stride, dtype=torch.float32, device=gout.device)
        H.call("smsut_scale", gx, gout.contiguous(), scale, out, gx.numel(), _s())
        return out, None


def mean_all(x, sign=1.0):
    return ScaledSumFn.apply(x, sign / x.numel())


class L1MeanFn(Function):

    @staticmethod
    def forward(ctx, a, b):
        a, b = nhwc(a), nhwc(b)
        out = torch.empty(1, dtype=torch.float32, device=a.device)
        n = a.numel()
        H.call("smsut_l1_fwd", a, b, out, _ws(H.call("smsut_sum_ws", n, 1), a), n, _s())
        ctx.save_for_backward(a, b)
        return out[0]

    @staticmethod
    @once_differentiable
    def backward(ctx, gout):
        a, b = ctx.saved_tensors
        ga = new_act(*a.shape, a) if ctx.needs_input_grad[0] else None
        gb = new_act(*b.shape, b) if ctx.needs_input_grad[1] else None
        if ga is not None or gb is not None:
            H.call("smsut_l1_bwd", a, b, gout.contiguous(), ga, gb, a.numel(), _s())
        return ga, gb


def l1_mean(a, b):
    return L1MeanFn.apply(a, b)


class SoftmaxMSEFn(Function):

    @staticmethod
    def forward(ctx, a, b):
        a, b = nhwc(a), nhwc(b)
        assert a.shape == b.shape
        n, c, h, w = a.shape
        out = torch.empty(1, dtype=torch.float32, device=a.device)
        H.call("smsut_softmax_mse_fwd", a, b, out, _ws(H.call("smsut_sum_ws", n * h * w, 1), a), n * h * w, c, _s())
        ctx.save_for_backward(a, b)
        return out[0]

    @staticmethod
    @once_differentiable
    def backward(ctx, gout):
        a, b = ctx.saved_tensors
        n, c, h, w = a.shape
        ga = new_act(n, c, h, w, a)
        H.call("smsut_softmax_mse_bwd", a, b, gout.contiguous().reshape(1), ga, n * h * w, c, _s())
        return ga, None


def softmax_mse(a, b):
    return SoftmaxMSEFn.apply(cl(a), cl(b).detach())


def argmax_channels(logits):
    z = nhwc(logits.detach())
    n, c, h, w = z.shape
    out = torch.empty(n, h, w, dtype=torch.int64, device=z.device)
    H.call("smsut_argmax_channels", z, out, n * h * w, c, _s())
    return out


EVAL_MAX_CLASSES, EVAL_MAX_SLICES = 32, 65535


def eval_overlap(logits, labels, vol_ids, counts, classes=None, want_pred=True):
    for what, t, dt in (("logits", logits, torch.float32), ("labels", labels, torch.int64), ("counts", counts, torch.int64)):
        if not isinstance(t, torch.Tensor):
            raise TypeError(f"eval_overlap: {what} must be a tensor, got {type(t).__name__}")
        if t.dtype != dt:
            raise TypeError(f"eval_overlap: {what} must be {dt}, got {t.dtype}")
        if not t.is_cuda or t.device != logits.device:
            raise TypeError(f"eval_overlap: {what} must be on the logits' HIP device, got {t.device} (no CPU fallback)")
    if logits.dim() != 4:
        raise ValueError(f"eval_overlap: expected NCHW logits, got shape {tuple(logits.shape)}")
    n, c, h, w = logits.shape
    k = c if classes is None else int(classes)
    if not 1 <= k <= min(c, EVAL_MAX_CLASSES):
        raise ValueError(f"eval_overlap: classes must lie in 1..min(C, {EVAL_MAX_CLASSES}), got {k} with C = {c}")
    if tuple(labels.shape) != (n, h, w):
        raise ValueError(f"eval_overlap: labels must be [N, H, W] = {(n, h, w)}, got {tuple(labels.shape)}")
    if counts.dim() != 3 or counts.shape[0] < 1 or tuple(counts.shape[1:]) != (k, 3) or not counts.is_contiguous():
        raise ValueError(f"eval_overlap: counts must be a contiguous [V >= 1, {k}, 3] tensor, got {tuple(counts.shape)}")
    if n > EVAL_MAX_SLICES or h * w < 1:
        raise ValueError(f"eval_overlap: needs at most {EVAL_MAX_SLICES} slices of at least one pixel, got {(n, h, w)}")
    ids = [int(i) for i in vol_ids]
    if len(ids) != n:
        raise ValueError(f"eval_overlap: {len(ids)} volume ids for {n} slices")
    n_vol = counts.shape[0]
    for i in ids:
        if not -1 <= i < n_vol:
            raise ValueError(f"eval_overlap: volume id {i} is neither -1 nor a slot of counts ({n_vol} slots)")
    pred = torch.empty(n, h, w, dtype=torch.uint8, device=logits.device) if want_pred else None
    if n == 0:
        return pred
    z = nhwc(logits.detach())
    vol = torch.tensor(ids, dtype=torch.int32).pin_memory().to(z.device, non_blocking=True)
    H.call("smsut_eval_overlap", z, labels.contiguous(), vol, counts, pred, n, h * w, c, k, n_vol, _s())
    return pred


def _cora_heads(logits, what):
    c = logits.shape[1]
    if c < 4 or (c - 1) % 3:
        raise ValueError(f"{what}: expected 3L+1 channels, got {c}")
    return (c - 1) // 3


def _cora_weights(w, n_cls, like):
    if w.dtype != torch.float32 or w.numel() != n_cls or w.device != like.device:
        raise ValueError(f"class weights must be {n_cls} fp32 values on {like.device}")
    return w.contiguous()


def _cora_labels(t, logits, dtype, what):
    n, _, h, w = logits.shape
    if t.dtype != dtype or tuple(t.shape) != (n, h, w):
        raise TypeError(f"{what} must be {dtype} of shape {(n, h, w)}, got {t.dtype} {tuple(t.shape)}")
    return t.contiguous()


def cora_sup_stats(logits, labels, w_con, w_rad):
    logits = nhwc(logits.detach())
    L = _cora_heads(logits, "cora_sup_stats")
    n, c, h, w = logits.shape
    labels = _cora_labels(labels, logits, torch.int64, "labels")
    stats = torch.empty(3 * (L + 1) + 3, dtype=torch.float32, device=logits.device)
    H.call("smsut_cora_sup_stats", logits, labels, _cora_weights(w_con, L + 1, logits), _cora_weights(w_rad, L + 1, logits), stats,
           _ws(H.call("smsut_cora_ws", n, h * w, L), logits), n, h * w, L, _s())
    return stats


class CoraSupFromStatsFn(Function):

    @staticmethod
    def forward(ctx, logits, labels, stats, w_con, w_rad, w_ce, w_dc, world):
        logits = nhwc(logits)
        L = _cora_heads(logits, "cora_sup_loss")
        n, c, h, w = logits.shape
        npix = float(n * h * w) * world
        w_con, w_rad = _cora_weights(w_con, L + 1, logits), _cora_weights(w_rad, L + 1, logits)
        out = torch.empty(4, dtype=torch.float32, device=logits.device)
        H.call("smsut_cora_sup_final", stats, w_con, w_rad, out, L, npix, float(w_dc), float(w_ce), _s())
        ctx.save_for_backward(logits, _cora_labels(labels, logits, torch.int64, "labels"), stats, w_con, w_rad)
        ctx.cfg = (L, npix, float(w_dc), float(w_ce), int(world))
        return out

    @staticmethod
    @once_differentiable
    def backward(ctx, gout):
        logits, labels, stats, w_con, w_rad = ctx.saved_tensors
        L, npix, w_dc, w_ce, world = ctx.cfg
        n, c, h, w = logits.shape
        gl = new_act(n, c, h, w, logits)
        gout = gout.contiguous()
        if world > 1:
            gout = gout * float(world)
        H.call("smsut_cora_sup_bwd", logits, labels, stats, w_con, w_rad, gout, gl, n, h * w, L, npix, w_dc, w_ce, _s())
        return gl, None, None, None, None, None, None, None


def cora_sup_loss(logits, labels, w_con, w_rad, weight_ce, weight_dc, group=None):
    stats = cora_sup_stats(logits, labels, w_con, w_rad)
    world = 1
    if group is not None:
        import torch.distributed as dist
        world = dist.get_world_size(group)
        if world > 1:
            all_reduce_dice_stats([(stats,)], group)
    return CoraSupFromStatsFn.apply(logits, labels, stats, w_con, w_rad, weight_ce, weight_dc, world)


class CoraSemiFn(Function):

    @staticmethod
    def forward(ctx, z, e, plab, mask, cw):
        z, e = nhwc(z), nhwc(e)
        if z.shape != e.shape:
            raise ValueError(f"student / teacher logits differ in shape: {tuple(z.shape)} vs {tuple(e.shape)}")
        L = _cora_heads(z, "cora_semi_loss")
        n, c, h, w = z.shape
        plab = _cora_labels(plab, z, torch.int64, "pseudo labels")
        mask = _cora_labels(mask, z, torch.float32, "mask")
        stats = torch.empty(n, 3 * (L + 1) + 4, dtype=torch.float32, device=z.device)
        H.call("smsut_cora_semi_stats", z, e, plab, mask, stats, _ws(H.call("smsut_cora_ws", n, h * w, L), z), n, h * w, L, _s())
        out = torch.empty(2, dtype=torch.float32, device=z.device)
        H.call("smsut_cora_semi_final", stats, out, n, L, float(cw), _s())
        ctx.save_for_backward(z, e, plab, mask, stats)
        ctx.cfg = (L, float(cw))
        return out

    @staticmethod
    @once_differentiable
    def backward(ctx, gout):
# ... 767 lines not shown
```

smsut-medicalimgsegmentation_amd/profiling.py:

```python
from __future__ import annotations

import collections
from typing import Callable, Dict, List, Tuple

import torch

from . import _hip as H


def _k2(ints, i):
    return ints[i] * ints[i]


_CONV_FLOPS: Dict[str, Tuple[Callable[[List[int]], float], str]] = {
    "smsut_conv2d_fwd_generic": (lambda a: 2.0 * a[0] * a[4] * a[5] * a[3] * a[6] * a[7] * a[8], "direct"),
    "smsut_conv2d_dgrad_generic": (lambda a: 2.0 * a[0] * a[4] * a[5] * a[3] * a[6] * a[7] * a[8], "direct"),
    "smsut_conv2d_wgrad_generic": (lambda a: 2.0 * a[0] * a[4] * a[5] * a[3] * a[6] * a[7] * a[8], "direct"),
    "smsut_conv2d_fwd_mfma": (lambda a: 2.0 * a[0] * a[1] * a[2] * a[3] * a[4] * _k2(a, 5), "mfma"),
    "smsut_conv2d_wgrad_pair": (lambda a: 2.0 * (a[0] + a[1]) * a[3] * a[4] * a[5] * a[6] * 9, "mfma"),
    "smsut_conv2d_wgrad_pair_slabs": (lambda a: 2.0 * (a[0] + a[1]) * a[2] * a[3] * a[4] * a[5] * 9, "mfma"),
    "smsut_conv2d_fwd_mfma_stats": (lambda a: 2.0 * a[0] * a[1] * a[2] * a[3] * a[4] * _k2(a, 5), "mfma"),
    "smsut_conv2d_dgrad_mfma_bwdstats": (lambda a: 2.0 * a[0] * a[1] * a[2] * a[3] * a[4] * 9, "mfma"),
    "smsut_conv2d_wgrad_mfma": (lambda a: 2.0 * a[0] * a[1] * a[2] * a[3] * a[4] * _k2(a, 5), "mfma"),
    "smsut_conv2d_fwd_mfma_stats_inaff": (lambda a: 2.0 * a[0] * a[1] * a[2] * a[3] * a[4] * 9, "mfma"),
    "smsut_conv2d_wgrad_mfma_inaff": (lambda a: 2.0 * a[0] * a[1] * a[2] * a[3] * a[4] * 9, "mfma"),
    "smsut_conv2d_wgrad_mfma_slabs": (lambda a: 2.0 * a[0] * a[1] * a[2] * a[3] * a[4] * 9, "mfma"),
    "smsut_conv2d_fwd_mfma_stats_cat": (lambda a: 2.0 * a[0] * a[1] * a[2] * a[3] * a[4] * 9, "mfma"),
    "smsut_conv2d_wgrad_mfma_cat": (lambda a: 2.0 * a[1] * a[2] * a[3] * a[4] * a[5] * _k2(a, 6), "mfma"),
    "smsut_conv2d_fwd_mfma_split": (lambda a: 2.0 * a[1] * a[2] * a[3] * a[4] * a[5] * 9, "mfma"),
    "smsut_conv2d_fwd_mfma_stats_sc": (lambda a: 2.0 * a[0] * a[1] * a[2] * a[3] * a[4] * 10, "mfma"),
    "smsut_conv2d_dgrad_mfma_sc": (lambda a: 2.0 * a[1] * a[2] * a[3] * a[4] * a[5] * 10, "mfma"),
    "smsut_conv2d_wgrad_mfma_sc": (lambda a: 2.0 * a[1] * a[2] * a[3] * a[4] * a[5] * 10, "mfma"),
    "smsut_conv2d_k4_fwd": (lambda a: 32.0 * a[0] * (a[1] - 1) * (a[2] - 1) * a[3] * a[4], "mfma"),
    "smsut_conv2d_k4_wgrad": (lambda a: 32.0 * a[0] * (a[1] - 1) * (a[2] - 1) * a[3] * a[4], "mfma"),
    "smsut_conv2d_fwd_mfma_f16": (lambda a: 2.0 * a[0] * a[1] * a[2] * a[3] * a[4] * _k2(a, 5), "mfma"),
    "smsut_conv2d_fwd_mfma_stats_f16": (lambda a: 2.0 * a[0] * a[1] * a[2] * a[3] * a[4] * _k2(a, 5), "mfma"),
    "smsut_conv2d_fwd_mfma_stats_cat_f16": (lambda a: 2.0 * a[0] * a[1] * a[2] * a[3] * a[4] * 9, "mfma"),
    "smsut_conv2d_fwd_mfma_stats_sc_f16": (lambda a: 2.0 * a[0] * a[1] * a[2] * a[3] * a[4] * 10, "mfma"),
    "smsut_conv2d_fwd_mfma_split_f16": (lambda a: 2.0 * a[1] * a[2] * a[3] * a[4] * a[5] * 9, "mfma"),
    "smsut_conv2d_dgrad_mfma_bwdstats_f16": (lambda a: 2.0 * a[0] * a[1] * a[2] * a[3] * a[4] * 9, "mfma"),
    "smsut_conv2d_wgrad_f16": (lambda a: 2.0 * a[1] * a[2] * a[3] * a[4] * a[5] * 9, "mfma"),
    "smsut_conv2d_dgrad_mfma_sc_f16": (lambda a: 2.0 * a[1] * a[2] * a[3] * a[4] * a[5] * 10, "mfma"),
    "smsut_conv2d_fwd_mfma_stats_f16_hs": (lambda a: 2.0 * a[0] * a[1] * a[2] * a[3] * a[4] * 9, "mfma"),
    "smsut_conv2d_fwd_mfma_stats_sc_f16_hs": (lambda a: 2.0 * a[0] * a[1] * a[2] * a[3] * a[4] * 10, "mfma"),
    "smsut_conv2d_fwd_mfma_stats_f16_hsx": (lambda a: 2.0 * a[0] * a[1] * a[2] * a[3] * a[4] * 9, "mfma"),
    "smsut_conv2d_wgrad_f16_xh": (lambda a: 2.0 * a[0] * a[1] * a[2] * a[3] * a[4] * 9, "mfma"),
    "smsut_conv2d_wgrad_f16_xh_inaff": (lambda a: 2.0 * a[0] * a[1] * a[2] * a[3] * a[4] * 9, "mfma"),
    "smsut_conv2d_fwd_mfma_stats_inaff_f16_hsx": (lambda a: 2.0 * a[0] * a[1] * a[2] * a[3] * a[4] * 9, "mfma"),
    "smsut_conv2d_dgrad_mfma_bwdstats_f16_hs": (lambda a: 2.0 * a[0] * a[1] * a[2] * a[3] * a[4] * 9, "mfma"),
    "smsut_conv2d_wgrad_sc_f16": (lambda a: 2.0 * a[1] * a[2] * a[3] * a[4] * a[5] * 10, "mfma"),
    "smsut_conv1x1_fwd": (lambda a: 2.0 * a[0] * a[1] * a[2] * a[3], "mfma"),
    "smsut_conv1x1_wgrad": (lambda a: 2.0 * a[0] * a[1] * a[2] * a[3], "mfma"),
    "smsut_conv1x1_fwd_cat": (lambda a: 2.0 * a[1] * a[2] * a[3] * a[4], "mfma"),
    "smsut_conv1x1_wgrad_cat": (lambda a: 2.0 * a[1] * a[2] * a[3] * a[4], "mfma"),
    "smsut_conv1x1_fwd_split": (lambda a: 2.0 * a[1] * a[2] * a[3] * a[4], "mfma"),
    "smsut_conv1x1_thin_dgrad": (lambda a: 2.0 * a[0] * a[1] * a[2] * a[3], "direct"),
    "smsut_conv1x1_thin_wgrad": (lambda a: 2.0 * a[0] * a[1] * a[2] * a[3], "direct"),
    "smsut_conv2d_small_fwd": (lambda a: 2.0 * a[0] * a[4] * a[5] * a[3] * a[6] * _k2(a, 7), "direct"),
    "smsut_conv2d_small_dgrad": (lambda a: 2.0 * a[0] * a[4] * a[5] * a[3] * a[6] * _k2(a, 7), "direct"),
    "smsut_conv2d_flat_wgrad": (lambda a: 2.0 * a[0] * a[4] * a[5] * a[3] * a[6] * _k2(a, 7), "mfma"),
    "smsut_convT2x2_fwd_mfma": (lambda a: 8.0 * a[0] * a[1] * a[2] * a[3] * a[4], "mfma"),
    "smsut_convT2x2_dgrad_mfma": (lambda a: 8.0 * a[0] * a[1] * a[2] * a[3] * a[4], "mfma"),
    "smsut_convT2x2_wgrad_mfma": (lambda a: 8.0 * a[0] * a[1] * a[2] * a[3] * a[4], "mfma"),
    "smsut_convT2x2_fwd_ps": (lambda a: 8.0 * a[0] * a[1] * a[2] * a[3] * a[4], "mfma"),
    "smsut_convT2x2_wgrad_ps": (lambda a: 8.0 * a[0] * a[1] * a[2] * a[3] * a[4], "mfma"),
}


_WINO = 16.0 / 36.0
_FORM: Dict[str, Tuple[Callable[[List[int]], Tuple[int, int, int, int, int, int]], float]] = {
    "smsut_conv2d_fwd_mfma": (lambda a: (a[0], a[1], a[2], a[3], a[4], 0) if a[5] == 3 else None, _WINO),
    "smsut_conv2d_fwd_mfma_stats": (lambda a: (a[0], a[1], a[2], a[3], a[4], 0) if a[5] == 3 else None, _WINO),
    "smsut_conv2d_dgrad_mfma_bwdstats": (lambda a: (a[0], a[1], a[2], a[3], a[4], 0), _WINO),
    "smsut_conv2d_fwd_mfma_stats_inaff": (lambda a: (a[0], a[1], a[2], a[3], a[4], 0), _WINO),
    "smsut_conv2d_fwd_mfma_stats_cat": (lambda a: (a[0], a[1], a[2], a[3], a[4], 0), _WINO),
    "smsut_conv2d_fwd_mfma_split": (lambda a: (a[1], a[2], a[3], a[4], a[5], 0) if a[6] == 3 else None, _WINO),
    "smsut_conv2d_fwd_mfma_stats_sc": (lambda a: (a[0], a[1], a[2], a[3], a[4], 0), 0.5),
    "smsut_conv2d_dgrad_mfma_sc": (lambda a: (a[1], a[2], a[3], 2 * a[4], a[5], 1), 0.8),
}


def _base(name: str) -> str:
    if name.endswith("_pre"):
        return name[:-4]
    if name.endswith("_fin"):
        return name[:-4]
    return name[:-5] if name.endswith("_amax") else name



def _ints(name: str, conv_args) -> List[int]:
    sig = H.SIGNATURES[name].replace(" ", "")
    return [a for c, a in zip(sig, conv_args) if c in "il"]


def executed_factor(name: str, conv_args) -> float:
    ent = _FORM.get(_base(name))
    if ent is None:
        return 1.0
    q = ent[0](_ints(name, conv_args))
    if q is None or H.call("smsut_conv2d_mfma_form", *q) == 0:
        return 1.0
    return ent[1]


def _pair_dims(conv_args):
    na, nb, _ca, h, w, cin, cout = [a for c, a in zip(H.SIGNATURES["smsut_conv2d_wgrad_pair"].replace(" ", ""), conv_args) if c == "i"]
    return na + nb, h, w, cin, cout, (10 if conv_args[3] is not None else 9)


def conv_flops_of(name: str, conv_args) -> float:
    if name == "smsut_conv2d_wgrad_pair":
        n, h, w, cin, cout, rows = _pair_dims(conv_args)
        return 2.0 * n * h * w * cin * cout * rows
    ent = _CONV_FLOPS.get(_base(name))
    if ent is None:
        return 0.0
    sig = H.SIGNATURES[name].replace(" ", "")
    ints = [a for c, a in zip(sig, conv_args) if c in "il"]
    return float(ent[0](ints))


def _cv(n, h, w, cin, cout, extra_out=0, extra_in=0):
    return 4.0 * n * h * w * (cin + extra_in + cout + extra_out)


_BYTES: Dict[str, Callable[[List[int]], float]] = {
    "smsut_conv2d_fwd_mfma": lambda a: _cv(a[0], a[1], a[2], a[3], a[4]),
    "smsut_conv2d_fwd_mfma_stats": lambda a: _cv(a[0], a[1], a[2], a[3], a[4]),
    "smsut_conv2d_dgrad_mfma_bwdstats": lambda a: _cv(a[0], a[1], a[2], a[3], a[4], extra_in=a[4]),
    "smsut_conv2d_fwd_mfma_stats_inaff": lambda a: _cv(a[0], a[1], a[2], a[3], a[4]),
    "smsut_conv2d_fwd_mfma_stats_cat": lambda a: _cv(a[0], a[1], a[2], a[3], a[4]),
    "smsut_conv2d_fwd_mfma_split": lambda a: _cv(a[1], a[2], a[3], a[4], a[5]),
    "smsut_conv2d_fwd_mfma_stats_sc": lambda a: _cv(a[0], a[1], a[2], a[3], a[4], extra_out=a[4]),
    "smsut_conv2d_fwd_mfma_stats_sc_f16": lambda a: _cv(a[0], a[1], a[2], a[3], a[4], extra_out=a[4]),
    "smsut_conv2d_dgrad_mfma_sc": lambda a: _cv(a[1], a[2], a[3], 2 * a[4], a[5]),
    "smsut_conv2d_dgrad_mfma_sc_f16": lambda a: _cv(a[1], a[2], a[3], 2 * a[4], a[5]),
    "smsut_conv2d_wgrad_sc_f16": lambda a: _cv(a[1], a[2], a[3], a[4], 2 * a[5]),
    "smsut_conv2d_wgrad_mfma": lambda a: _cv(a[0], a[1], a[2], a[3], a[4]),
    "smsut_conv2d_wgrad_mfma_inaff": lambda a: _cv(a[0], a[1], a[2], a[3], a[4]),
    "smsut_conv2d_wgrad_mfma_cat": lambda a: _cv(a[1], a[2], a[3], a[4], a[5]),
    "smsut_conv2d_wgrad_mfma_sc": lambda a: _cv(a[1], a[2], a[3], a[4], 2 * a[5]),
    "smsut_conv1x1_fwd": lambda a: 4.0 * a[0] * a[1] * (a[2] + a[3]),
    "smsut_conv1x1_wgrad": lambda a: 4.0 * a[0] * a[1] * (a[2] + a[3]),
    "smsut_convT2x2_fwd_mfma": lambda a: 4.0 * a[0] * a[1] * a[2] * (a[3] + 4 * a[4]),
    "smsut_convT2x2_dgrad_mfma": lambda a: 4.0 * a[0] * a[1] * a[2] * (a[3] + 4 * a[4]),
    "smsut_convT2x2_wgrad_mfma": lambda a: 4.0 * a[0] * a[1] * a[2] * (a[3] + 4 * a[4]),
    "smsut_convT2x2_fwd_ps": lambda a: 4.0 * a[0] * a[1] * a[2] * (a[3] + 4 * a[4]),
    "smsut_convT2x2_wgrad_ps": lambda a: 4.0 * a[0] * a[1] * a[2] * (a[3] + 4 * a[4]),
    "smsut_restail_fwd": lambda a: 4.0 * a[0] * a[1] * a[2] * 3,
    "smsut_restail_bwd": lambda a: 4.0 * a[0] * a[1] * a[2] * 5,
    "smsut_in_apply_bwd": lambda a: 4.0 * a[0] * a[1] * a[2] * 3,
    "smsut_instnorm_fwd": lambda a: 4.0 * a[0] * a[1] * a[2] * 2,
    "smsut_instnorm_fwd_partials": lambda a: 4.0 * a[1] * a[2] * a[3] * 2,
    "smsut_instnorm_bwd": lambda a: 4.0 * a[0] * a[1] * a[2] * 3,
    "smsut_instnorm_bwd2": lambda a: 4.0 * a[0] * a[1] * a[2] * 5,
    "smsut_restail_fwd_pool": lambda a: a[0] * a[1] * a[2] * a[3] * ((2.0 * 2 if a[4] else 4.0 * 2) + 4.0 * 1.25 + 0.25),
    "smsut_restail_bwd_pool": lambda a: a[0] * a[1] * a[2] * a[3] * ((2.0 * 2 if a[4] else 4.0 * 2) + 4.0 * 3.25 + 0.25),
    "smsut_instnorm_pool_fwd_partials": lambda a: 4.0 * a[1] * a[2] * a[3] * a[4] * 1.25,
    "smsut_instnorm_pool_bwd": lambda a: 4.0 * a[0] * a[1] * a[2] * a[3] * 2.25,
    "smsut_maxpool2_fwd": lambda a: 4.0 * a[0] * a[1] * a[2] * a[3] * 1.25,
    "smsut_maxpool2_bwd": lambda a: 4.0 * a[0] * a[1] * a[2] * a[3] * 2.25,
    "smsut_maxpool2_bwd_add": lambda a: 4.0 * a[0] * a[1] * a[2] * a[3] * 3.25,
    "smsut_avgpool2_fwd": lambda a: 4.0 * a[0] * a[1] * a[2] * a[3] * 1.25,
    "smsut_avgpool2_bwd": lambda a: 4.0 * a[0] * a[1] * a[2] * a[3] * 1.25,
    "smsut_add_act": lambda a: 4.0 * a[0] * 3,
    "smsut_conv2d_fwd_mfma_stats_f16_hs": lambda a: a[0] * a[1] * a[2] * (4.0 * a[3] + 2.0 * a[4]),
    "smsut_conv2d_fwd_mfma_stats_sc_f16_hs": lambda a: a[0] * a[1] * a[2] * (4.0 * a[3] + 2.0 * 2 * a[4]),
    "smsut_conv2d_dgrad_mfma_bwdstats_f16_hs": lambda a: a[0] * a[1] * a[2] * (4.0 * a[3] + 4.0 * a[4] + 2.0 * a[4]),
    "smsut_restail_fwd_hs": lambda a: a[0] * a[1] * a[2] * (2.0 * 2 + 4.0),
    "smsut_restail_bwd_hs": lambda a: a[0] * a[1] * a[2] * (4.0 * 3 + 2.0 * 2),
    "smsut_in_apply_bwd_hs": lambda a: a[0] * a[1] * a[2] * (4.0 * 2 + 2.0),
    "smsut_instnorm_fwd_partials_hs": lambda a: a[1] * a[2] * a[3] * (2.0 + 4.0),
    "smsut_instnorm_fwd_partials_hs2": lambda a: a[1] * a[2] * a[3] * (2.0 + 2.0),
    "smsut_conv2d_fwd_mfma_stats_f16_hsx": lambda a: a[0] * a[1] * a[2] * (2.0 * a[3] + 2.0 * a[4]),
    "smsut_conv2d_wgrad_f16_xh": lambda a: a[0] * a[1] * a[2] * (2.0 * a[3] + 4.0 * a[4]),
    "smsut_conv2d_wgrad_f16_xh_inaff": lambda a: a[0] * a[1] * a[2] * (2.0 * a[3] + 4.0 * a[4]),
    "smsut_conv2d_fwd_mfma_stats_inaff_f16_hsx": lambda a: a[0] * a[1] * a[2] * (2.0 * a[3] + 2.0 * a[4]),
    "smsut_act_bwd": lambda a: 4.0 * a[0] * 3,
    "smsut_tanh_fwd": lambda a: 4.0 * a[0] * 2,
    "smsut_tanh_bwd": lambda a: 4.0 * a[0] * 3,
    "smsut_edt_sq": lambda a: a[0] * a[2] * a[3] * (8.0 + 4.0 * a[1] + 2.0 * a[1] / 8.0),
    "smsut_sdf_final": lambda a: a[0] * a[2] * a[3] * (8.0 + 4.0 * a[1] + 4.0 * a[1]),
    "smsut_dtc_loss_fwd": lambda a: 4.0 * a[2] * a[3] * (2 * a[0] + a[1]),
    "smsut_dtc_loss_bwd": lambda a: 4.0 * a[2] * a[3] * (4 * a[0] + a[1]),
}


def bytes_of(name: str, conv_args) -> float:
    if name == "smsut_conv2d_wgrad_pair":
        n, h, w, cin, cout, rows = _pair_dims(conv_args)
        return _cv(n, h, w, cin, cout * (2 if rows == 10 else 1))
    ent = _BYTES.get(_base(name))
    return float(ent(_ints(name, conv_args))) if ent else 0.0


def _byte_class(name: str) -> str:
    n = _base(name)
    if "conv" in n:
        return "convolutions"
    if "restail" in n:
        return "residual tails"
    if "instnorm" in n or "in_apply" in n:
        return "InstanceNorm"
    return "pooling / pointwise"


class Row(collections.namedtuple("Row", "name args calls us flops exec_flops abytes")):
    @property
    def total_us(self):
        return self.us * self.calls


_NO_REPLAY = {"smsut_sgd_momentum_multi"}


def record_step(step: Callable[[], object]):
    rec = []
    orig = H.call

    def spy(name, *args):
        if name not in H._NO_STATUS and name not in _NO_REPLAY:
            rec.append((name, [H.ptr(a) if isinstance(a, torch.Tensor) or a is None else a for a in args]))
        return orig(name, *args)
    H.call = spy
    try:
        step()
        torch.cuda.synchronize()
    finally:
        H.call = orig
    return rec



def replay(rec, reps: int = 8) -> List[Row]:
    lib = H.load()
    groups = collections.OrderedDict()
    for name, conv in rec:
        sig = H.SIGNATURES[name].replace(" ", "")
        key = (name, tuple(a for c, a in zip(sig, conv) if c in "ilfd"))
        groups.setdefault(key, []).append(conv)
    e0, e1 = torch.cuda.Event(enable_timing=True), torch.cuda.Event(enable_timing=True)
    st = torch.cuda.current_stream()
    rows = []
    for (name, shp), calls in groups.items():
        conv = list(calls[0])
        fn = getattr(lib, name)
        conv[-1] = st.cuda_stream
        for _ in range(2):
            fn(*conv)
        torch.cuda.synchronize()
        e0.record(st)
        for _ in range(reps):
            fn(*conv)
        e1.record(st)
        torch.cuda.synchronize()
        fl = conv_flops_of(name, calls[0])
        rows.append(Row(name, shp, len(calls), e0.elapsed_time(e1) / reps * 1e3, fl, fl * executed_factor(name, calls[0]),
                        bytes_of(name, calls[0])))
    return rows


def summarize(rows: List[Row], peak_tflops: float) -> dict:
    conv = [r for r in rows if r.flops > 0]
    mfma = [r for r in conv if _CONV_FLOPS[_base(r.name)][1] == "mfma"]
    t_all = sum(r.total_us for r in rows)
    t_conv = sum(r.total_us for r in conv)
    f_conv = sum(r.flops * r.calls for r in conv)
    x_conv = sum(r.exec_flops * r.calls for r in conv)
    t_mfma = sum(r.total_us for r in mfma)
    f_mfma = sum(r.flops * r.calls for r in mfma)
    x_mfma = sum(r.exec_flops * r.calls for r in mfma)
    fam = collections.OrderedDict()
    for r in conv:
        k = ("wgrad" if "wgrad" in r.name else "fwd/dgrad") + (" 1x1" if "1x1" in r.name else (" convT" if "convT" in r.name else ""))
        t, f, x = fam.get(k, (0.0, 0.0, 0.0))
        fam[k] = (t + r.total_us, f + r.flops * r.calls, x + r.exec_flops * r.calls)
    byc = collections.OrderedDict()
    for r in rows:
        if r.abytes > 0:
            k = _byte_class(r.name)
            t, b = byc.get(k, (0.0, 0.0))
            byc[k] = (t + r.total_us, b + r.abytes * r.calls)
    tf = lambda f, t: round(f / (t * 1e-6) / 1e12, 2) if t else None
    fr = lambda f, t: round(f / (t * 1e-6) / 1e12 / peak_tflops, 4) if t else None
    return {
        "kernel_ms_all": round(t_all / 1e3, 3), "kernel_ms_conv": round(t_conv / 1e3, 3),
        "conv_gflop": round(f_conv / 1e9, 2), "conv_gflop_mfma_executed": round(x_conv / 1e9, 2),
        "step_conv_tflops": tf(f_conv, t_conv), "step_conv_frac": fr(f_conv, t_conv),
        "step_conv_tflops_mfma_executed": tf(x_conv, t_conv), "step_conv_frac_mfma_executed": fr(x_conv, t_conv),
        "mfma_conv_frac_algorithmic": fr(f_mfma, t_mfma), "mfma_conv_frac_executed": fr(x_mfma, t_mfma),
        "conv_share_of_kernel_time": round(t_conv / t_all, 4) if t_all else None,
        "algorithmic_gbytes": round(sum(b for _, b in byc.values()) / 1e9, 3),
        "algorithmic_bytes_by_class": {k: {"gbytes": round(b / 1e9, 3), "ms": round(t / 1e3, 3), "gbs": round(b / (t * 1e-6) / 1e9, 1)}
                                       for k, (t, b) in byc.items()},
        "families": {k: {"ms": round(t / 1e3, 3), "algorithmic_tflops": round(f / (t * 1e-6) / 1e12, 1),
                         "mfma_executed_tflops": round(x / (t * 1e-6) / 1e12, 1)} for k, (t, f, x) in fam.items()},
    }


def table(rows: List[Row], min_share: float = 0.007) -> str:
    tot = sum(r.total_us for r in rows) or 1.0
    out = []
    for r in sorted(rows, key=lambda r: -r.total_us):
        if r.total_us / tot < min_share:
            break
        tf = f"{r.flops / (r.us * 1e-6) / 1e12:6.1f} TF" if r.flops else "         "
        out.append(f"{r.total_us / 1e3:7.3f} ms {100 * r.total_us / tot:5.1f}%  {r.calls:3d} x {r.us:7.1f} us {tf}  "
                   f"{r.name.replace('smsut_', '')} {r.args}")
    return "\n".join(out)


def lost_table(rows: List[Row], peak_tflops: float) -> str:
    tot = sum(r.total_us for r in rows) or 1.0
    ent = []
    for r in rows:
        ideal = r.flops / (peak_tflops * 1e12) * 1e6 if r.flops else 0.0
        ent.append((r.total_us - ideal * r.calls, r))
    out = []
    for lost, r in sorted(ent, key=lambda e: -e[0]):
        tf = f"{r.flops / (r.us * 1e-6) / 1e12:6.1f} TF" if r.flops else "         "
        out.append(f"lost {lost / 1e3:7.3f} ms  total {r.total_us / 1e3:7.3f} ms {100 * r.total_us / tot:5.1f}%  {r.calls:3d} x {r.us:7.1f} us {tf}  "
                   f"{r.name.replace('smsut_', '')} {r.args}")
    return "\n".join(out)
```

Before: 829.7.

## Fold per-sample modality planes into stem conv via border-class bias tables

The TSL encoder's first 5x5 conv no longer gets its input from materialised constant modality planes concatenated to the image. Because each modality channel is constant per sample, its contribution is precomputed as a small 5x5 table of per-border-class offsets and added to a 1-channel conv. Dgrad reads only the image-channel weights, and wgrad reduces the modality-channel gradients from row and column sums of gy. This removes the plane-building kernel, the wide input channels and the channel-copy in backward, at the cost of more specialised kernels and edge-class logic that could go wrong at borders.

```diff
diff --git a/include/smsut_hip.h b/include/smsut_hip.h
--- a/include/smsut_hip.h
+++ b/include/smsut_hip.h
@@ -198,6 +198,14 @@
 int64_t smsut_conv2d_flat_wgrad_ws(int N, int Ho, int Wo, int Cin, int Cout, int KS);
 int smsut_conv2d_flat_wgrad(const float* x, const float* gy, float* gw, float* workspace, int N, int H, int W, int Cin,
                             int Ho, int Wo, int Cout, int KS, int stride, int pad, void* stream);
+
+int smsut_stem_modal_supported(int H, int W, int M);
+int smsut_stem_modal_fwd(const float* x, const float* m, const float* w, const float* bias, float* y, int N, int H, int W, int M,
+                         void* stream);
+int smsut_stem_modal_dgrad(const float* gy, const float* w, float* gx, int N, int H, int W, int M, void* stream);
+int64_t smsut_stem_modal_wgrad_ws(int N, int H, int W, int M);
+int smsut_stem_modal_wgrad(const float* x, const float* m, const float* gy, float* gw, float* workspace, int N, int H, int W, int M,
+                           void* stream);
 
 int smsut_convT2x2_mfma_supported(int Cin, int Cout);
 int smsut_convT2x2_fwd_mfma(const float* x, const float* w, float* y, int N, int H, int W, int Cin, int Cout, void* stream);
diff --git a/profiles/stem_modal_step.py b/profiles/stem_modal_step.py
--- /dev/null
+++ b/profiles/stem_modal_step.py
@@ -0,0 +1,100 @@
+#!/usr/bin/env python3
+import argparse
+import json
+import os
+import sys
+
+ROOT = os.path.dirname(os.path.dirname(os.path.abspath(__file__)))
+sys.path.insert(0, ROOT)
+
+
+def main():
+    ap = argparse.ArgumentParser()
+    ap.add_argument("--n", type=int, default=16)
+    ap.add_argument("--size", type=int, default=256)
+    ap.add_argument("--modal", type=int, default=4)
+    ap.add_argument("--kernels", action="store_true")
+    ap.add_argument("--iters", type=int, default=200)
+    ap.add_argument("--rounds", type=int, default=5)
+    args = ap.parse_args()
+
+    import torch
+    import smsut_amd
+    from smsut_amd import _hip as H
+    if not torch.cuda.is_available():
+        raise SystemExit("profiles/stem_modal_step.py measures on the GPU; none is visible")
+    n, s, m_planes = args.n, args.size, args.modal
+    cw = 1 + m_planes
+    g = torch.Generator().manual_seed(3)
+    x = torch.randn(n, s, s, 1, generator=g).cuda()
+    m = torch.zeros(n, m_planes)
+    m[torch.arange(n), torch.arange(n) % m_planes] = 1.0
+    m = m.cuda()
+    w = (torch.randn(5, 5, cw, 8, generator=g) * (25 * cw) ** -0.5).cuda()
+    gy = torch.randn(n, s, s, 8, generator=g).cuda()
+    full, y_old, y_new = torch.empty(n, s, s, cw).cuda(), torch.empty(n, s, s, 8).cuda(), torch.empty(n, s, s, 8).cuda()
+    gfull, gx_old, gx_new = torch.empty(n, s, s, cw).cuda(), torch.empty(n, s, s, 1).cuda(), torch.empty(n, s, s, 1).cuda()
+    gw_old, gw_new = torch.empty(5, 5, cw, 8).cuda(), torch.empty(5, 5, cw, 8).cuda()
+    ws_old = torch.empty(H.call("smsut_conv2d_flat_wgrad_ws", n, s, s, cw, 8, 5)).cuda()
+    ws_new = torch.empty(H.call("smsut_stem_modal_wgrad_ws", n, s, s, m_planes)).cuda()
+    st = H.stream_ptr()
+
+    def fwd_old():
+        H.call("smsut_modal_planes", x, m, full, n, s * s, 1, m_planes, st)
+        H.call("smsut_conv2d_small_fwd", full, w, None, y_old, n, s, s, cw, s, s, 8, 5, 1, 2, st)
+
+    def fwd_new():
+        H.call("smsut_stem_modal_fwd", x, m, w, None, y_new, n, s, s, m_planes, st)
+
+    def dgrad_old():
+        H.call("smsut_conv2d_small_dgrad", gy, w, gfull, n, s, s, cw, s, s, 8, 5, 1, 2, st)
+        H.call("smsut_copy_channels", gfull, cw, 0, gx_old, 1, 0, 1, n * s * s, st)
+
+    def dgrad_new():
+        H.call("smsut_stem_modal_dgrad", gy, w, gx_new, n, s, s, m_planes, st)
+
+    def wgrad_old():
+        H.call("smsut_conv2d_flat_wgrad", full, gy, gw_old, ws_old, n, s, s, cw, s, s, 8, 5, 1, 2, st)
+
+    def wgrad_new():
+        H.call("smsut_stem_modal_wgrad", x, m, gy, gw_new, ws_new, n, s, s, m_planes, st)
+
+    legs = {"fwd_old": fwd_old, "fwd_new": fwd_new, "dgrad_old": dgrad_old, "dgrad_new": dgrad_new, "wgrad_old": wgrad_old,
+            "wgrad_new": wgrad_new}
+    for fn in legs.values():
+        for _ in range(5):
+            fn()
+    torch.cuda.synchronize()
+
+    def rel(a, b):
+        return float((a - b).abs().max() / b.abs().max())
+    agree = {"y": rel(y_new, y_old), "gx": rel(gx_new, gx_old), "gw": rel(gw_new, gw_old)}
+    assert max(agree.values()) < 1e-5, agree
+
+    if args.kernels:
+        for fn in legs.values():
+            for _ in range(24):
+                fn()
+        torch.cuda.synchronize()
+        return
+
+    def timed(fn, iters):
+        a, b = torch.cuda.Event(enable_timing=True), torch.cuda.Event(enable_timing=True)
+        a.record()
+        for _ in range(iters):
+            fn()
+        b.record()
+        torch.cuda.synchronize()
+        return a.elapsed_time(b) / iters * 1e3
+
+    times = {k: [] for k in legs}
+    for _ in range(args.rounds):
+        for k, fn in legs.items():
+            times[k].append(round(timed(fn, args.iters), 2))
+    med = {k: sorted(v)[len(v) // 2] for k, v in times.items()}
+    print(json.dumps({"device": torch.cuda.get_device_name(0), "n": n, "size": s, "modal": m_planes, "max_rel_diff_new_vs_old": agree,
+                      "us_median": med, "us_all": times}))
+
+
+if __name__ == "__main__":
+    main()
diff --git a/smsut-medicalimgsegmentation_amd/_hip.py b/smsut-medicalimgsegmentation_amd/_hip.py
--- a/smsut-medicalimgsegmentation_amd/_hip.py
+++ b/smsut-medicalimgsegmentation_amd/_hip.py
@@ -142,6 +142,11 @@
     "smsut_conv2d_flat_wgrad_supported": "iiii",
     "smsut_conv2d_flat_wgrad_ws": "iiiiii",
     "smsut_conv2d_flat_wgrad": "pppp iiiiiiiiii s",
+    "smsut_stem_modal_supported": "iii",
+    "smsut_stem_modal_fwd": "ppppp iiii s",
+    "smsut_stem_modal_dgrad": "ppp iiii s",
+    "smsut_stem_modal_wgrad_ws": "iiii",
+    "smsut_stem_modal_wgrad": "ppppp iiii s",
     "smsut_add_act": "ppp l f s",
     "smsut_act_bwd": "ppp l f s",
     "smsut_tanh_fwd": "pp l s",
@@ -236,12 +241,12 @@
     "smsut_calibration_stats": "pppp iiiiii f s",
 }
 _RET_I64 = {"smsut_wino_image_floats", "smsut_conv2d_wgrad_pair_ws", "smsut_convT2x2_wgrad_ps_ws", "smsut_conv2d_wgrad_sc_ws", "smsut_conv2d_k4_wgrad_ws", "smsut_conv2d_wgrad_f16_ws", "smsut_conv2d_wgrad_sc_f16_ws", "smsut_absmax_scale_ws", "smsut_conv2d_wgrad_generic_ws", "smsut_colsum_ws", "smsut_dicece_ws", "smsut_sum_ws",
-            "smsut_conv2d_wgrad_mfma_ws", "smsut_convT2x2_wgrad_mfma_ws", "smsut_conv2d_flat_wgrad_ws", "smsut_conv1x1_wgrad_ws",
+            "smsut_conv2d_wgrad_mfma_ws", "smsut_convT2x2_wgrad_mfma_ws", "smsut_conv2d_flat_wgrad_ws", "smsut_stem_modal_wgrad_ws", "smsut_conv1x1_wgrad_ws",
             "smsut_conv1x1_thin_wgrad_ws", "smsut_cc_ws", "smsut_surface_ws", "smsut_surface_hd_ws", "smsut_surface_sp_ws", "smsut_surface_hd_sp_ws", "smsut_cora_ws",
             "smsut_sdf_ws", "smsut_dtc_ws", "smsut_image_similarity_ws",
             "smsut_bspline_ws", "smsut_resample_ws", "smsut_order_statistics_ws", "smsut_calibration_ws"}
 _NO_STATUS = _RET_I64 | {"smsut_conv2d_k4_supported", "smsut_conv2d_f16_supported", "smsut_conv2d_wgrad_f16_supported", "smsut_in_chunks", "smsut_in_slabs", "smsut_amax_blocks", "smsut_conv2d_mfma_supported", "smsut_conv2d_wgrad_mfma_supported",
-                         "smsut_convT2x2_mfma_supported", "smsut_conv2d_small_supported",
+                         "smsut_convT2x2_mfma_supported", "smsut_conv2d_small_supported", "smsut_stem_modal_supported",
                          "smsut_conv2d_flat_wgrad_supported", "smsut_conv2d_mfma_tiles", "smsut_conv2d_mfma_persistent", "smsut_conv1x1_supported",
                          "smsut_conv1x1_tiles", "smsut_conv1x1_thin_supported", "smsut_conv2d_mfma_split_supported", "smsut_conv2d_mfma_cat_supported",
                          "smsut_conv2d_fwd_sc_supported", "smsut_conv2d_fwd_sc_f16_supported", "smsut_conv2d_dgrad_sc_supported",
diff --git a/smsut-medicalimgsegmentation_amd/csrc/conv_small.hip b/smsut-medicalimgsegmentation_amd/csrc/conv_small.hip
--- a/smsut-medicalimgsegmentation_amd/csrc/conv_small.hip
+++ b/smsut-medicalimgsegmentation_amd/csrc/conv_small.hip
@@ -233,6 +233,41 @@
 }
 
 template <int CIN>
+__device__ __forceinline__ void stem_fwd_taps(const float* in_s, const float* w_s, const float* __restrict__ bias, int row, int cg,
+                                              float (&acc)[4][SCO]) {
+#pragma unroll
+  for (int p = 0; p < 4; ++p)
+#pragma unroll
+    for (int c = 0; c < SCO; ++c) acc[p][c] = bias ? bias[c] : 0.f;
+#pragma unroll
+  for (int kh = 0; kh < SKS; ++kh)
+#pragma unroll
+    for (int ci = 0; ci < CIN; ++ci) {
+      float v[8];
+      const float* ip = in_s + (ci * SIH + row + kh) * SIW + 4 * cg;
+      *(float4*)v = *(const float4*)ip; *(float4*)(v + 4) = *(const float4*)(ip + 4);
+#pragma unroll
+      for (int kw = 0; kw < SKS; ++kw) {
+        float wv[SCO];
+        const float* wp = w_s + ((kh * SKS + kw) * CIN + ci) * SCO;
+        *(float4*)wv = *(const float4*)wp; *(float4*)(wv + 4) = *(const float4*)(wp + 4);
+#pragma unroll
+        for (int p = 0; p < 4; ++p)
+#pragma unroll
+          for (int c = 0; c < SCO; ++c) acc[p][c] = fmaf(v[p + kw], wv[c], acc[p][c]);
+      }
+    }
+}
+
+__device__ __forceinline__ void stem_fwd_store(float* __restrict__ yp, float (&acc)[4][SCO]) {
+#pragma unroll
+  for (int p = 0; p < 4; ++p) {
+    *(float4*)(yp + p * SCO) = *(float4*)acc[p];
+    *(float4*)(yp + p * SCO + 4) = *(float4*)(acc[p] + 4);
+  }
+}
+
+template <int CIN>
 __global__ void __launch_bounds__(TPB)
 stem_fwd(const float* __restrict__ x, const float* __restrict__ w, const float* __restrict__ bias, float* __restrict__ y,
          int N, int H, int W) {
@@ -247,45 +282,72 @@
   __syncthreads();
   const int row = threadIdx.x >> 4, cg = threadIdx.x & 15;
   float acc[4][SCO];
-#pragma unroll
-  for (int p = 0; p < 4; ++p)
-#pragma unroll
-    for (int c = 0; c < SCO; ++c) acc[p][c] = bias ? bias[c] : 0.f;
-#pragma unroll
-  for (int kh = 0; kh < SKS; ++kh)
-#pragma unroll
-    for (int ci = 0; ci < CIN; ++ci) {
-      float v[8];
-      const float* ip = in_s + (ci * SIH + row + kh) * SIW + 4 * cg;
-      *(float4*)v = *(const float4*)ip; *(float4*)(v + 4) = *(const float4*)(ip + 4);
-#pragma unroll
-      for (int kw = 0; kw < SKS; ++kw) {
-        float wv[SCO];
-        const float* wp = w_s + ((kh * SKS + kw) * CIN + ci) * SCO;
-        *(float4*)wv = *(const float4*)wp; *(float4*)(wv + 4) = *(const float4*)(wp + 4);
-#pragma unroll
-        for (int p = 0; p < 4; ++p)
-#pragma unroll
-          for (int c = 0; c < SCO; ++c) acc[p][c] = fmaf(v[p + kw], wv[c], acc[p][c]);
-      }
-    }
-  float* yp = y + (((size_t)n * H + y0 + row) * W + x0 + 4 * cg) * SCO;
+  stem_fwd_taps<CIN>(in_s, w_s, bias, row, cg, acc);
+  stem_fwd_store(y + (((size_t)n * H + y0 + row) * W + x0 + 4 * cg) * SCO, acc);
+}
+
+constexpr int SMM = 4;
+__device__ __forceinline__ int stem_class(int i, int n) { return i < 2 ? i : (i >= n - 2 ? i - (n - 5) : 2); }
+__device__ __forceinline__ int stem_tap_lo(int a) { return a < 2 ? 2 - a : 0; }
+__device__ __forceinline__ int stem_tap_hi(int a) { return a > 2 ? 6 - a : 4; }
+
+__global__ void __launch_bounds__(TPB)
+stem_modal_fwd(const float* __restrict__ x, const float* __restrict__ m, const float* __restrict__ w, const float* __restrict__ bias,
+               float* __restrict__ y, int N, int H, int W, int M) {
+  __shared__ __attribute__((aligned(16))) float in_s[SIH * SIW];
+  __shared__ __attribute__((aligned(16))) float w_s[SKS * SKS * SCO];
+  __shared__ __attribute__((aligned(16))) float wm_s[SKS * SKS * SMM * SCO];
+  __shared__ __attribute__((aligned(16))) float t_s[5 * 5 * SCO];
+  const int tiles_x = W / STX, tiles_y = H / STY;
+  const int t = blockIdx.x;
+  const int n = t / (tiles_x * tiles_y), rem = t % (tiles_x * tiles_y);
+  const int y0 = (rem / tiles_x) * STY, x0 = (rem % tiles_x) * STX;
+  const int cw = 1 + M;
+  for (int u = threadIdx.x; u < SKS * SKS * cw * SCO; u += TPB) {
+    const int tap = u / (cw * SCO), ch = (u / SCO) % cw, co = u % SCO;
+    if (ch == 0) w_s[tap * SCO + co] = w[u];
+    else wm_s[(tap * SMM + ch - 1) * SCO + co] = w[u];
+  }
+  stem_stage<1>(x, in_s, n, y0, x0, H, W);
+  __syncthreads();
+  if (threadIdx.x < 5 * 5 * SCO) {
+    const int a = threadIdx.x / (5 * SCO), b = (threadIdx.x / SCO) % 5, co = threadIdx.x % SCO;
+    float mj[SMM];
+#pragma unroll
+    for (int j = 0; j < SMM; ++j) mj[j] = j < M ? m[(size_t)n * M + j] : 0.f;
+    float s = 0.f;
+    for (int kh = stem_tap_lo(a); kh <= stem_tap_hi(a); ++kh)
+      for (int kw = stem_tap_lo(b); kw <= stem_tap_hi(b); ++kw)
+#pragma unroll
+        for (int j = 0; j < SMM; ++j)
+          if (j < M) s = fmaf(mj[j], wm_s[((kh * SKS + kw) * SMM + j) * SCO + co], s);
+    t_s[threadIdx.x] = s;
+  }
+  const int row = threadIdx.x >> 4, cg = threadIdx.x & 15;
+  float acc[4][SCO];
+  stem_fwd_taps<1>(in_s, w_s, bias, row, cg, acc);
+  __syncthreads();
+  const int ra = stem_class(y0 + row, H);
 #pragma unroll
   for (int p = 0; p < 4; ++p) {
-    *(float4*)(yp + p * SCO) = *(float4*)acc[p];
-    *(float4*)(yp + p * SCO + 4) = *(float4*)(acc[p] + 4);
-  }
+    const float* tp = t_s + (ra * 5 + stem_class(x0 + 4 * cg + p, W)) * SCO;
+    float tv[SCO];
+    *(float4*)tv = *(const float4*)tp; *(float4*)(tv + 4) = *(const float4*)(tp + 4);
+#pragma unroll
+    for (int c = 0; c < SCO; ++c) acc[p][c] += tv[c];
+  }
+  stem_fwd_store(y + (((size_t)n * H + y0 + row) * W + x0 + 4 * cg) * SCO, acc);
 }
 
 __global__ void __launch_bounds__(TPB)
-stem_dgrad1(const float* __restrict__ gy, const float* __restrict__ w, float* __restrict__ gx, int N, int H, int W) {
+stem_dgrad1(const float* __restrict__ gy, const float* __restrict__ w, float* __restrict__ gx, int N, int H, int W, int cw) {
   __shared__ __attribute__((aligned(16))) float g_s[SCO * SIH * SIW];
   __shared__ __attribute__((aligned(16))) float w_s[SKS * SKS * SCO];
   const int tiles_x = W / STX, tiles_y = H / STY;
   const int t = blockIdx.x;
   const int n = t / (tiles_x * tiles_y), rem = t % (tiles_x * tiles_y);
   const int y0 = (rem / tiles_x) * STY, x0 = (rem % tiles_x) * STX;
-  for (int u = threadIdx.x; u < SKS * SKS * SCO; u += TPB) w_s[u] = w[u];
+  for (int u = threadIdx.x; u < SKS * SKS * SCO; u += TPB) w_s[u] = w[(u / SCO) * cw * SCO + u % SCO];
   for (int u = threadIdx.x; u < SIH * SIW * 2; u += TPB) {
     const int h = u & 1, pix = u >> 1;
     const int iy = pix / SIW, ix = pix % SIW;
@@ -316,15 +378,17 @@
 }
 
 constexpr int SGQ = 36;
-template <int CIN>
+template <int CIN, bool MODAL = false>
 __global__ void __launch_bounds__(TPB)
 stem_wgrad(const float* __restrict__ x, const float* __restrict__ gy, float* __restrict__ part, int N, int H, int W,
-           int tiles_per_wg) {
+           int tiles_per_wg, const float* __restrict__ m, int M) {
+  static_assert(!MODAL || CIN == 1, "the modal form stages the image channel alone");
   extern __shared__ __attribute__((aligned(16))) float smem[];
   float* in_s = smem;
   float* gy_s = smem + CIN * SIH * SIW;
   constexpr int NACC = SKS * SCO;
   constexpr int TPP = (CIN == 1) ? 32 : 8;
+  const int CW = MODAL ? 1 + M : CIN;
   const int tiles_x = W / STX, tiles_y = H / STY, total = N * tiles_x * tiles_y;
   const int q = threadIdx.x / TPP, sub = threadIdx.x % TPP;
   const bool live = q < SKS * CIN;
@@ -332,6 +396,14 @@
   float acc[NACC];
 #pragma unroll
   for (int i = 0; i < NACC; ++i) acc[i] = 0.f;
+  const int ml = threadIdx.x - 3 * 64, mco = ml & 7, mpx = (ml >> 3) & 3, mrh = ml >> 5;
+  float macc[SMM][3][2];
+  if constexpr (MODAL) {
+#pragma unroll
+    for (int j = 0; j < SMM; ++j)
+#pragma unroll
+      for (int r = 0; r < 3; ++r) macc[j][r][0] = macc[j][r][1] = 0.f;
+  }
   const int t0 = blockIdx.x * tiles_per_wg, t1 = min(t0 + tiles_per_wg, total);
   for (int t = t0; t < t1; ++t) {
     const int n = t / (tiles_x * tiles_y), rem = t % (tiles_x * tiles_y);
@@ -367,6 +439,39 @@
         }
       }
     }
+    if constexpr (MODAL) {
+      if (ml >= 0) {
+        const bool cedge = mpx < 2 ? x0 == 0 : x0 + STX == W;
+        const bool redge = mrh == 0 ? y0 == 0 : y0 + STY == H;
+        const float* gp = gy_s + mrh * 8 * (STX / 4) * SGQ + mpx * SCO + mco;
+        float s[3][2];
+#pragma unroll
+        for (int r = 0; r < 3; ++r) s[r][0] = s[r][1] = 0.f;
+#pragma unroll
+        for (int r = 0; r < 8; ++r) {
+          float inner = 0.f;
+#pragma unroll
+          for (int qd = 1; qd < STX / 4 - 1; ++qd) inner += gp[(r * (STX / 4) + qd) * SGQ];
+          const float first = gp[r * (STX / 4) * SGQ], last = gp[(r * (STX / 4) + STX / 4 - 1) * SGQ];
+          float edge = mpx < 2 ? first : last;
+          inner += mpx < 2 ? last : first;
+          if (!cedge) { inner += edge; edge = 0.f; }
+          const bool b0 = redge && r == (mrh == 0 ? 0 : 6), b1 = redge && r == (mrh == 0 ? 1 : 7);
+          s[0][0] += b0 || b1 ? 0.f : inner; s[0][1] += b0 || b1 ? 0.f : edge;
+          s[1][0] += b0 ? inner : 0.f;       s[1][1] += b0 ? edge : 0.f;
+          s[2][0] += b1 ? inner : 0.f;       s[2][1] += b1 ? edge : 0.f;
+        }
+#pragma unroll
+        for (int j = 0; j < SMM; ++j) {
+          const float mj = j < M ? m[(size_t)n * M + j] : 0.f;
+#pragma unroll
+          for (int r = 0; r < 3; ++r) {
+            macc[j][r][0] = fmaf(mj, s[r][0], macc[j][r][0]);
+            macc[j][r][1] = fmaf(mj, s[r][1], macc[j][r][1]);
+          }
+        }
+      }
+    }
   }
 #pragma unroll
   for (int i = 0; i < NACC; ++i) {
@@ -375,12 +480,47 @@
     if constexpr (TPP == 32) { a += __shfl_xor(a, 8, 64); a += __shfl_xor(a, 16, 64); }
     acc[i] = a;
   }
+  float* out = part + (size_t)blockIdx.x * SKS * SKS * CW * SCO;
   if (live && sub == 0) {
-    float* out = part + (size_t)blockIdx.x * SKS * SKS * CIN * SCO;
 #pragma unroll
     for (int kw = 0; kw < SKS; ++kw)
 #pragma unroll
-      for (int c = 0; c < SCO; ++c) out[((kh * SKS + kw) * CIN + k2) * SCO + c] = acc[kw * SCO + c];
+      for (int c = 0; c < SCO; ++c) out[((kh * SKS + kw) * CW + k2) * SCO + c] = acc[kw * SCO + c];
+  }
+  if constexpr (MODAL) {
+    float* lane_s = smem;
+    float* cls_s = smem + SMM * 6 * 64;
+    __syncthreads();
+    if (ml >= 0) {
+#pragma unroll
+      for (int j = 0; j < SMM; ++j)
+#pragma unroll
+        for (int r = 0; r < 3; ++r) {
+          lane_s[((j * 3 + r) * 2 + 0) * 64 + ml] = macc[j][r][0];
+          lane_s[((j * 3 + r) * 2 + 1) * 64 + ml] = macc[j][r][1];
+        }
+    }
+    __syncthreads();
+    for (int u = threadIdx.x; u < M * 5 * 5 * SCO; u += TPB) {
+      const int j = u / (5 * 5 * SCO), a = (u / (5 * SCO)) % 5, b = (u / SCO) % 5, co = u % SCO;
+      const int r = a == 2 ? 0 : (a == 0 || a == 3 ? 1 : 2);
+      const int rh0 = a <= 2 ? 0 : 1, rh1 = a >= 2 ? 1 : 0;
+      const int px0 = b == 2 ? 0 : (b < 2 ? b : b - 1), px1 = b == 2 ? 3 : px0;
+      const float* ls = lane_s + ((j * 3 + r) * 2 + (b == 2 ? 0 : 1)) * 64 + co;
+      float v = 0.f;
+      for (int rh = rh0; rh <= rh1; ++rh)
+        for (int px = px0; px <= px1; ++px) v += ls[rh * 32 + px * SCO];
+      cls_s[u] = v;
+    }
+    __syncthreads();
+    for (int u = threadIdx.x; u < SKS * SKS * M * SCO; u += TPB) {
+      const int tap = u / (M * SCO), j = (u / SCO) % M, co = u % SCO;
+      const int th = tap / SKS, tw = tap % SKS;
+      float v = 0.f;
+      for (int a = stem_tap_lo(th); a <= stem_tap_hi(th); ++a)
+        for (int b = stem_tap_lo(tw); b <= stem_tap_hi(tw); ++b) v += cls_s[((j * 5 + a) * 5 + b) * SCO + co];
+      out[(tap * CW + 1 + j) * SCO + co] = v;
+    }
   }
 }
 
@@ -388,9 +528,10 @@
   return g.KS == SKS && g.stride == 1 && g.pad == SPD && g.Cout == SCO && (g.Cin == 1 || g.Cin == 5) && g.H % STY == 0 &&
          g.W % STX == 0 && g.Ho == g.H && g.Wo == g.W;
 }
+constexpr int STEM_WGS_CAP = 512;
 inline int stem_wgrad_wgs(const SmallGeom& g, int max_slabs) {
   const int total = g.N * (g.H / STY) * (g.W / STX);
-  int wgs = total < 512 ? total : 512;
+  int wgs = total < STEM_WGS_CAP ? total : STEM_WGS_CAP;
   if (wgs > max_slabs) wgs = max_slabs;
   return wgs < 1 ? 1 : wgs;
 }
@@ -453,7 +594,7 @@
   const int grid = ew_grid(npix) * 2;
   hipStream_t st = (hipStream_t)stream;
   if (stem_shape(g) && Cin == 1) {
-    stem_dgrad1<<<N * (H / STY) * (W / STX), TPB, 0, st>>>(gy, w, gx, N, H, W);
+    stem_dgrad1<<<N * (H / STY) * (W / STX), TPB, 0, st>>>(gy, w, gx, N, H, W, 1);
     SMSUT_LAUNCH_CHECK();
     return SMSUT_OK;
   }
@@ -494,12 +635,12 @@
     const int wsz = KS * KS * Cin * Cout;
     if (Cin == 1) {
       constexpr size_t sh = (size_t)(1 * SIH * SIW + STY * (STX / 4) * SGQ) * sizeof(float);
-      stem_wgrad<1><<<nwg, TPB, sh, st>>>(x, gy, workspace, N, H, W, tpw);
+      stem_wgrad<1><<<nwg, TPB, sh, st>>>(x, gy, workspace, N, H, W, tpw, nullptr, 0);
     } else {
       constexpr size_t sh = (size_t)(5 * SIH * SIW + STY * (STX / 4) * SGQ) * sizeof(float);
       static bool attr = false;
       if (!attr) { (void)hipFuncSetAttribute((const void*)stem_wgrad<5>, hipFuncAttributeMaxDynamicSharedMemorySize, (int)sh); attr = true; }
-      stem_wgrad<5><<<nwg, TPB, sh, st>>>(x, gy, workspace, N, H, W, tpw);
+      stem_wgrad<5><<<nwg, TPB, sh, st>>>(x, gy, workspace, N, H, W, tpw, nullptr, 0);
     }
     flat_sum<<<(wsz + FS_COLS - 1) / FS_COLS, TPB, 0, st>>>(workspace, gw, wsz, nwg);
     SMSUT_LAUNCH_CHECK();
@@ -516,4 +657,45 @@
   return SMSUT_OK;
 }
 
-}
+int smsut_stem_modal_supported(int H, int W, int M) {
+  return H >= STY && W >= STX && H % STY == 0 && W % STX == 0 && M >= 1 && M <= SMM;
+}
+
+int smsut_stem_modal_fwd(const float* x, const float* m, const float* w, const float* bias, float* y, int N, int H, int W, int M,
+                         void* stream) {
+  SMSUT_REQUIRE(x && m && w && y && N > 0 && smsut_stem_modal_supported(H, W, M));
+  stem_modal_fwd<<<N * (H / STY) * (W / STX), TPB, 0, (hipStream_t)stream>>>(x, m, w, bias, y, N, H, W, M);
+  SMSUT_LAUNCH_CHECK();
+  return SMSUT_OK;
+}
+
+int smsut_stem_modal_dgrad(const float* gy, const float* w, float* gx, int N, int H, int W, int M, void* stream) {
+  SMSUT_REQUIRE(gy && w && gx && N > 0 && smsut_stem_modal_supported(H, W, M));
+  stem_dgrad1<<<N * (H / STY) * (W / STX), TPB, 0, (hipStream_t)stream>>>(gy, w, gx, N, H, W, 1 + M);
+  SMSUT_LAUNCH_CHECK();
+  return SMSUT_OK;
+}
+
+int64_t smsut_stem_modal_wgrad_ws(int N, int H, int W, int M) {
+  SmallGeom g{N, H, W, 1, H, W, SCO, SKS, 1, SPD};
+  return (int64_t)stem_wgrad_wgs(g, STEM_WGS_CAP) * SKS * SKS * (1 + M) * SCO;
+}
+
+int smsut_stem_modal_wgrad(const float* x, const float* m, const float* gy, float* gw, float* workspace, int N, int H, int W, int M,
+                           void* stream) {
+  SMSUT_REQUIRE(x && m && gy && gw && workspace && N > 0 && smsut_stem_modal_supported(H, W, M));
+  SmallGeom g{N, H, W, 1, H, W, SCO, SKS, 1, SPD};
+  const int wgs = stem_wgrad_wgs(g, STEM_WGS_CAP);
+  const int total = N * (H / STY) * (W / STX);
+  const int tpw = (total + wgs - 1) / wgs;
+  const int nwg = (total + tpw - 1) / tpw;
+  const int wsz = SKS * SKS * (1 + M) * SCO;
+  constexpr size_t sh = (size_t)(1 * SIH * SIW + STY * (STX / 4) * SGQ) * sizeof(float);
+  hipStream_t st = (hipStream_t)stream;
+  stem_wgrad<1, true><<<nwg, TPB, sh, st>>>(x, gy, workspace, N, H, W, tpw, m, M);
+  flat_sum<<<(wsz + FS_COLS - 1) / FS_COLS, TPB, 0, st>>>(workspace, gw, wsz, nwg);
+  SMSUT_LAUNCH_CHECK();
+  return SMSUT_OK;
+}
+
+}
diff --git a/smsut-medicalimgsegmentation_amd/network/ugan.py b/smsut-medicalimgsegmentation_amd/network/ugan.py
--- a/smsut-medicalimgsegmentation_amd/network/ugan.py
+++ b/smsut-medicalimgsegmentation_amd/network/ugan.py
@@ -11,8 +11,14 @@
 
 class _Pre(nn.Sequential):
 
-    def forward(self, x):
-        return self[1](self[0](x, stats=True), slope=self[2].slope)
+    def forward(self, x, m=None):
+        if m is None:
+            y = self[0](x, stats=True)
+        elif ops.modal_stem_supported(x, m, self[0]):
+            y = ops.modal_stem(x, m, self[0])
+        else:
+            y = self[0](ops.modal_planes(x, m), stats=True)
+        return self[1](y, slope=self[2].slope)
 
 
 class Encoder(nn.Module):
@@ -26,9 +32,9 @@
             setattr(self, f"enc{i}", BasicBlock(chans[i - 1], chans[i], norm_type, act_type))
             setattr(self, f"pool{i}", MaxPool2x2())
 
-    def forward(self, x):
+    def forward(self, x, m=None):
         skips = []
-        x = self.pre(x)
+        x = self.pre(x, m)
         for i in range(1, 5):
             x, skip = encoder_level(getattr(self, f"enc{i}"), getattr(self, f"pool{i}"), x)
             skips.append(skip)
@@ -78,8 +84,7 @@
     def _tsl_branch(self, x, m):
         if m is None:
             m = torch.zeros(x.size(0), self.n_modal, device=x.device)
-        tsl_in = ops.modal_planes(x, m.to(x.device))
-        t_bot, t_sk = self.tsl_encoder(tsl_in)
+        t_bot, t_sk = self.tsl_encoder(x, m.to(x.device))
         t_e5 = self.enc5(t_bot)
         return self.tsl_decoder(t_e5, t_sk), t_e5
 
diff --git a/smsut-medicalimgsegmentation_amd/ops.py b/smsut-medicalimgsegmentation_amd/ops.py
--- a/smsut-medicalimgsegmentation_amd/ops.py
+++ b/smsut-medicalimgsegmentation_amd/ops.py
@@ -1626,6 +1626,57 @@
     return ModalPlanesFn.apply(x, m)
 
 
+MODAL_STEM = bool(int(_os.environ.get("SMSUT_MODAL_STEM", "1")))
+
+
+def modal_stem_supported(x, m, conv):
+    if not MODAL_STEM or CONV_F16 or x.dim() != 4 or m.dim() != 2 or x.dtype != torch.float32:
+        return False
+    w = conv.weight
+    n, cx, h, wd = x.shape
+    return (cx == 1 and m.shape[0] == n and tuple(w.shape) == (8, 1 + m.shape[1], 5, 5) and conv.stride == 1 and conv.padding == 2
+            and bool(H.call("smsut_stem_modal_supported", h, wd, m.shape[1])))
+
+
+class ModalStemFn(Function):
+
+    @staticmethod
+    def forward(ctx, x, m, w, bias):
+        x, w = nhwc(x), hwio(w)
+        n, _, h, wd = x.shape
+        m = m.detach().to(torch.float32).contiguous()
+        nm = m.shape[1]
+        y = new_act(n, w.shape[0], h, wd, x)
+        H.call("smsut_stem_modal_fwd", x, m, w, bias, y, n, h, wd, nm, _s())
+        ctx.save_for_backward(x, m, w)
+        ctx.has_bias = bias is not None
+        return y
+
+    @staticmethod
+    @once_differentiable
+    def backward(ctx, gy):
+        x, m, w = ctx.saved_tensors
+        gy = nhwc(gy)
+        n, _, h, wd = x.shape
+        nm = m.shape[1]
+        gx = gw = gb = None
+        if ctx.needs_input_grad[0]:
+            gx = new_act(n, 1, h, wd, gy)
+            H.call("smsut_stem_modal_dgrad", gy, w, gx, n, h, wd, nm, _s())
+        if not _INPUT_GRADS_ONLY:
+            if ctx.needs_input_grad[2]:
+                gw = new_weight(w.shape[0], 1 + nm, 5, 5, device=x.device)
+                ws = _ws(H.call("smsut_stem_modal_wgrad_ws", n, h, wd, nm), x)
+                H.call("smsut_stem_modal_wgrad", x, m, gy, gw, ws, n, h, wd, nm, _s())
+            if ctx.has_bias and ctx.needs_input_grad[3]:
+                gb = SumPerChannelFn.apply(gy)
+        return gx, None, gw, gb
+
+
+def modal_stem(x, m, conv):
+    return ModalStemFn.apply(cl(x), m, conv.weight, conv.bias)
+
+
 def dice_ce_stats(logits, labels, batch_dice):
     logits = nhwc(logits.detach())
     n, c, h, w = logits.shape
diff --git a/smsut-medicalimgsegmentation_amd/profiling.py b/smsut-medicalimgsegmentation_amd/profiling.py
--- a/smsut-medicalimgsegmentation_amd/profiling.py
+++ b/smsut-medicalimgsegmentation_amd/profiling.py
@@ -59,6 +59,9 @@
     "smsut_conv2d_small_fwd": (lambda a: 2.0 * a[0] * a[4] * a[5] * a[3] * a[6] * _k2(a, 7), "direct"),
     "smsut_conv2d_small_dgrad": (lambda a: 2.0 * a[0] * a[4] * a[5] * a[3] * a[6] * _k2(a, 7), "direct"),
     "smsut_conv2d_flat_wgrad": (lambda a: 2.0 * a[0] * a[4] * a[5] * a[3] * a[6] * _k2(a, 7), "mfma"),
+    "smsut_stem_modal_fwd": (lambda a: 2.0 * a[0] * a[1] * a[2] * (1 + a[3]) * 8 * 25, "direct"),
+    "smsut_stem_modal_dgrad": (lambda a: 2.0 * a[0] * a[1] * a[2] * 1 * 8 * 25, "direct"),
+    "smsut_stem_modal_wgrad": (lambda a: 2.0 * a[0] * a[1] * a[2] * (1 + a[3]) * 8 * 25, "direct"),
     "smsut_convT2x2_fwd_mfma": (lambda a: 8.0 * a[0] * a[1] * a[2] * a[3] * a[4], "mfma"),
     "smsut_convT2x2_dgrad_mfma": (lambda a: 8.0 * a[0] * a[1] * a[2] * a[3] * a[4], "mfma"),
     "smsut_convT2x2_wgrad_mfma": (lambda a: 8.0 * a[0] * a[1] * a[2] * a[3] * a[4], "mfma"),
@@ -141,6 +144,9 @@
     "smsut_conv2d_wgrad_mfma_inaff": lambda a: _cv(a[0], a[1], a[2], a[3], a[4]),
     "smsut_conv2d_wgrad_mfma_cat": lambda a: _cv(a[1], a[2], a[3], a[4], a[5]),
     "smsut_conv2d_wgrad_mfma_sc": lambda a: _cv(a[1], a[2], a[3], a[4], 2 * a[5]),
+    "smsut_stem_modal_fwd": lambda a: _cv(a[0], a[1], a[2], 1, 8),
+    "smsut_stem_modal_dgrad": lambda a: _cv(a[0], a[1], a[2], 1, 8),
+    "smsut_stem_modal_wgrad": lambda a: _cv(a[0], a[1], a[2], 1, 8),
     "smsut_conv1x1_fwd": lambda a: 4.0 * a[0] * a[1] * (a[2] + a[3]),
     "smsut_conv1x1_wgrad": lambda a: 4.0 * a[0] * a[1] * (a[2] + a[3]),
     "smsut_convT2x2_fwd_mfma": lambda a: 4.0 * a[0] * a[1] * a[2] * (a[3] + 4 * a[4]),
@@ -197,7 +203,7 @@
 
 def _byte_class(name: str) -> str:
     n = _base(name)
-    if "conv" in n:
+    if "conv" in n or "stem_modal" in n:
         return "convolutions"
     if "restail" in n:
         return "residual tails"
```

Result: no change. 834.4 (median of 6 runs) (+0.6%).
